# TACC/GraviT

Hardware: AMD Instinct MI355X
Metric: Mrays/s (primary+shadow) at 1080p, 10M-tri scene (higher is better)
Workload: dtype f32; 1 GPU; soup-10000000: 10000000 random triangles (Philox seed 12345, half-extent 0.005), 1920x1080, eye (.5,.5,3)->(.5,.5,.5), fov 30deg, 1 point light at the eye, depth 1 (primary + 1 shadow ray), AO off; scheduler=image, 1 domain, harness=native, settle_frames=0, normal_mode=flat

## Files before the change

### gravit_amd/capi.py

```python
import ctypes as C
import os

import numpy as np

from .layouts import HIT_DTYPE, LIGHT_DTYPE, MATERIAL_DTYPE, RAY_DTYPE

HERE = os.path.dirname(os.path.abspath(__file__))
LIB_PATH = os.environ.get("GVT_HIP_LIB") or os.path.join(HERE, "libgvt_hip.so")

ABI_VERSION = 6

SYMBOLS = [
    "gvt_hip_init", "gvt_hip_set_stream", "gvt_hip_synchronize", "gvt_hip_last_error",
    "gvt_hip_mesh_create", "gvt_hip_mesh_destroy", "gvt_hip_trace_ex", "gvt_hip_mesh_get_info", "gvt_hip_mesh_get_normals", "gvt_hip_mesh_update_vertices",
    "gvt_hip_trace", "gvt_hip_intersect", "gvt_hip_occluded",
    "gvt_hip_queue_create", "gvt_hip_queue_destroy", "gvt_hip_queue_reserve", "gvt_hip_queue_clear", "gvt_hip_queue_size",
    "gvt_hip_queue_append", "gvt_hip_queue_append_flags", "gvt_hip_abi_version", "gvt_hip_queue_export", "gvt_hip_trace_queue", "gvt_hip_trace_queue_sink",
    "gvt_hip_camera_generate",
    "gvt_hip_camera_generate_tiled",
    "gvt_hip_camera_filter",
    "gvt_hip_top_create", "gvt_hip_top_destroy", "gvt_hip_top_order", "gvt_hip_top_update", "gvt_hip_shuffle", "gvt_hip_queue_sizes",
    "gvt_hip_fb_create", "gvt_hip_fb_destroy", "gvt_hip_fb_clear", "gvt_hip_fb_download", "gvt_hip_fb_device_ptr",
    "gvt_hip_fb_write_ppm_bytes",
    "gvt_hip_profile", "gvt_hip_stats_read", "gvt_hip_stats_reset", "gvt_hip_set_option", "gvt_hip_is_experiments_build", "gvt_hip_counters_peek", "gvt_hip_visit_stats", "gvt_hip_wide_visit_stats", "gvt_hip_mesh_download_nodes", "gvt_hip_mesh_download_wide", "gvt_hip_mesh_download_clusters", "gvt_hip_mesh_upload_nodes", "gvt_hip_marked_visit_stats", "gvt_hip_image_frame",
    "gvt_hip_math_probe", "gvt_hip_ctx_create", "gvt_hip_ctx_make_current", "gvt_hip_ctx_destroy",
    "gvt_hip_comm_unique_id", "gvt_hip_comm_create", "gvt_hip_hub_create", "gvt_hip_hub_abort", "gvt_hip_hub_destroy", "gvt_hip_comm_create_local",
    "gvt_hip_comm_destroy", "gvt_hip_comm_rank", "gvt_hip_comm_world", "gvt_hip_comm_count", "gvt_hip_comm_reserved_cus", "gvt_hip_comm_set_deadline_ms", "gvt_hip_comm_selftest",
    "gvt_hip_tracer_create", "gvt_hip_tracer_destroy", "gvt_hip_tracer_set_camera", "gvt_hip_tracer_set_transforms", "gvt_hip_tracer_set_domains", "gvt_hip_tracer_frame",
    "gvt_hip_volume_create", "gvt_hip_volume_destroy", "gvt_hip_volume_get_info", "gvt_hip_volume_set_transfer", "gvt_hip_volume_trace",
    "gvt_hip_shuffle_volume", "gvt_hip_volume_frame",
    "gvt_hip_volume_set_surfaces", "gvt_hip_volume_set_lights", "gvt_hip_volume_get_crossings",
    "gvt_hip_volume_set_shading", "gvt_hip_volume_get_shading", "gvt_hip_volume_get_shaded",
    "gvt_hip_volume_update_samples",
    "gvt_hip_volume_create_typed", "gvt_hip_volume_update_samples_typed", "gvt_hip_volume_get_voxel_type",
    "gvt_hip_depth_create", "gvt_hip_depth_destroy", "gvt_hip_depth_clear", "gvt_hip_depth_upload", "gvt_hip_depth_download", "gvt_hip_depth_render",
    "gvt_hip_volume_frame_clipped", "gvt_hip_fb_composite_over",
    "gvt_hip_volume_set_subgrids", "gvt_hip_volume_get_amr_info",
    "gvt_hip_volume_march_queue", "gvt_hip_volume_camera_filter", "gvt_hip_queues_export_wire", "gvt_hip_queues_append_wire",
    "gvt_hip_volume_set_ghosts", "gvt_hip_volume_set_gradient", "gvt_hip_volume_get_gradient",
    "gvt_hip_volume_frame_fused", "gvt_hip_volume_frame_fused_shaded", "gvt_hip_volume_frame_fused_amr",
    "gvt_hip_volume_frame_shadowed",
    "gvt_hip_volume_light_grid_bake", "gvt_hip_volume_light_grid_download", "gvt_hip_volume_light_grid_info", "gvt_hip_volume_light_grid_release",
    "gvt_hip_volume_frame_fog_shadowed",
    "gvt_hip_volume_occluder_grid_bake", "gvt_hip_volume_occluder_grid_download", "gvt_hip_volume_occluder_grid_info", "gvt_hip_volume_occluder_grid_release",
    "gvt_hip_volume_frame_mesh_shadowed",
]


class GvtHipError(RuntimeError):
    pass


class MeshInfo(C.Structure):
    _fields_ = [("n_tris", C.c_uint64), ("n_verts", C.c_uint64), ("n_nodes", C.c_uint64), ("n_leaves", C.c_uint64),
                ("bbox_lo", C.c_float * 3), ("bbox_hi", C.c_float * 3), ("build_ms", C.c_float), ("max_leaf", C.c_uint32),
                ("packet", C.c_uint32), ("bytes_nodes", C.c_uint64), ("bytes_tris", C.c_uint64), ("sah_inner", C.c_float), ("pad", C.c_float)]


class CameraPod(C.Structure):
    _fields_ = [("eye", C.c_float * 3), ("focus", C.c_float * 3), ("up", C.c_float * 3), ("fov", C.c_float), ("width", C.c_int32),
                ("height", C.c_int32), ("samples", C.c_int32), ("depth", C.c_int32), ("jitter_window_size", C.c_float)]


class FrameStats(C.Structure):
    _fields_ = [("rounds", C.c_uint64), ("chains", C.c_uint64), ("host_syncs", C.c_uint64), ("rays_sent", C.c_uint64),
                ("rays_closest", C.c_uint64), ("rays_any", C.c_uint64), ("packets_bailed", C.c_uint64), ("bytes_sent", C.c_uint64),
                ("ms_chain", C.c_double), ("ms_announce", C.c_double), ("ms_payload", C.c_double), ("ms_composite", C.c_double), ("ms_host_wait", C.c_double),
                ("exchanges", C.c_uint64), ("rays_inline", C.c_uint64), ("early_deposit_launches", C.c_uint64)]

    def as_dict(self):
        return {k: getattr(self, k) for k, _ in self._fields_}


class VolumeInfo(C.Structure):
    _fields_ = [("box_lo", C.c_float * 3), ("box_hi", C.c_float * 3), ("dt", C.c_float), ("value_min", C.c_float), ("value_max", C.c_float),
                ("blocks", C.c_int32 * 3), ("pad", C.c_float), ("n_blocks", C.c_uint64), ("n_blocks_empty", C.c_uint64),
                ("samples_marched", C.c_uint64), ("samples_gathered", C.c_uint64)]

    def as_dict(self):
        return {k: (list(getattr(self, k)) if k in ("box_lo", "box_hi", "blocks") else getattr(self, k)) for k, _ in self._fields_ if k != "pad"}


class SubgridPod(C.Structure):
    _fields_ = [("parent", C.c_int32), ("ratio", C.c_int32), ("lo", C.c_int32 * 3), ("cells", C.c_int32 * 3)]


class VolumeAmrInfo(C.Structure):
    _fields_ = [("n_subgrids", C.c_int32), ("n_levels", C.c_int32), ("subgrid_bytes", C.c_uint64), ("samples_refined", C.c_uint64),
                ("amr_marches", C.c_uint64)]

    def as_dict(self):
        return {k: getattr(self, k) for k, _ in self._fields_}


class VolumeFusedStats(C.Structure):
    _fields_ = [("fused", C.c_uint32), ("pad", C.c_uint32), ("samples_marched", C.c_uint64), ("samples_gathered", C.c_uint64),
                ("brick_visits", C.c_uint64), ("rays_deposited", C.c_uint64), ("adapter_calls", C.c_uint64)]

    def as_dict(self):
        return {k: getattr(self, k) for k, _ in self._fields_ if k != "pad"}


class VolumeFusedShadedStats(C.Structure):
    _fields_ = [("fused", C.c_uint32), ("features", C.c_uint32), ("samples_marched", C.c_uint64), ("samples_gathered", C.c_uint64),
                ("brick_visits", C.c_uint64), ("rays_deposited", C.c_uint64), ("adapter_calls", C.c_uint64), ("crossings_rendered", C.c_uint64),
                ("samples_shaded", C.c_uint64)]

    def as_dict(self):
        return {k: getattr(self, k) for k, _ in self._fields_}


class VolumeFusedAmrStats(C.Structure):
    _fields_ = VolumeFusedShadedStats._fields_ + [("samples_refined", C.c_uint64), ("amr_bricks", C.c_uint32), ("pad", C.c_uint32)]

    def as_dict(self):
        return {k: getattr(self, k) for k, _ in self._fields_ if k != "pad"}


class VolumeShadowParams(C.Structure):
    _fields_ = [("flags", C.c_uint32), ("bias", C.c_int32)]


class VolumeShadowStats(C.Structure):
    _fields_ = VolumeFusedShadedStats._fields_ + [("shadowed", C.c_uint32), ("pad", C.c_uint32), ("shadow_rays", C.c_uint64), ("shadow_brick_visits", C.c_uint64),
                                                  ("shadow_crossings", C.c_uint64), ("shadow_samples_marched", C.c_uint64), ("shadow_samples_gathered", C.c_uint64)]

    def as_dict(self):
        return {k: getattr(self, k) for k, _ in self._fields_ if k != "pad"}


class VolumeLightGridParams(C.Structure):
    _fields_ = [("flags", C.c_uint32), ("bias", C.c_int32)]


class VolumeLightGridStats(C.Structure):
    _fields_ = [("rays", C.c_uint64), ("samples_marched", C.c_uint64), ("samples_gathered", C.c_uint64), ("crossings", C.c_uint64), ("bytes", C.c_uint64),
                ("ms", C.c_float), ("pad", C.c_uint32)]

    def as_dict(self):
        return {k: getattr(self, k) for k, _ in self._fields_ if k != "pad"}


class VolumeLightGridState(C.Structure):
    _fields_ = [("present", C.c_uint32), ("current", C.c_uint32), ("n_planes", C.c_int32), ("bias", C.c_int32), ("bytes", C.c_uint64)]

    def as_dict(self):
        return {k: getattr(self, k) for k, _ in self._fields_}


class VolumeFogShadowStats(C.Structure):
    _fields_ = VolumeShadowStats._fields_ + [("fog_samples_shadowed", C.c_uint64)]
# ... 203 lines not shown
```

### gravit_amd/csrc/api.hip

```cpp
#include <atomic>
#include <chrono>
#include <cmath>
#include <cstdlib>
#include <condition_variable>
#include <functional>
#include <mutex>
#include <new>
#include <thread>

#include "gvt_internal.h"

size_t trav_spill_ints_per_thread();
int trav_block_threads();
void abi_pool_destroy(void *);

static thread_local std::string g_err;
static Ctx g_default_ctx;
static thread_local Ctx *tl_ctx = nullptr;
#define g_ctx (gctx())
Ctx &gctx() { return tl_ctx ? *tl_ctx : g_default_ctx; }

void set_error(const char *fmt, ...) {
  char buf[1024];
  va_list ap;
// ... 134 lines not shown
  C.scratch_bytes[slot] = want;
  return C.scratch[slot];
}

void scratch_release(ScratchSlot slot) {
  Ctx &C = g_ctx;
  if (!C.scratch[slot]) return;
  hipStreamSynchronize(C.stream);
  hipFree(C.scratch[slot]);
  C.scratch[slot] = nullptr;
  C.scratch_bytes[slot] = 0;
}

ProfScope::ProfScope(int c) : cls(c) {
  Ctx &C = g_ctx;
  if (!C.profile || (C.profile == 2 && c != KC_CLOSEST && c != KC_ANY && c != KC_LONG) || (C.profile == 3 && c != KC_CLOSEST) || (C.profile == 4 && c != KC_ANY)) return;
  auto take = [&]() {
    hipEvent_t e;
    if (!C.event_pool.empty()) { e = C.event_pool.back(); C.event_pool.pop_back(); }
    else hipEventCreate(&e);
    return e;
  };
  a = take(); b = take();
  hipEventRecord(a, C.stream);
}
ProfScope::~ProfScope() {
  Ctx &C = g_ctx;
  if (!a) return;
  hipEventRecord(b, C.stream);
  C.pending.push_back({ a, b, cls });
}
static void drain_events() {
  Ctx &C = g_ctx;
  for (auto &p : C.pending) {
    hipEventSynchronize(p.b);
    float ms = 0.f;
    hipEventElapsedTime(&ms, p.a, p.b);
    double *slot[KC_COUNT] = { &C.stats.ms_closest, &C.stats.ms_any, &C.stats.ms_shade, &C.stats.ms_convert, &C.stats.ms_shuffle,
                               &C.stats.ms_camera, &C.stats.ms_build, &C.stats.ms_sort, &C.stats.ms_long };
    *slot[p.cls] += ms;
    C.event_pool.push_back(p.a);
    C.event_pool.push_back(p.b);
  }
  C.pending.clear();
}
extern "C" int gvt_hip_profile(int enable) {
  if (ensure_init()) return GVT_HIP_ERR_NODEVICE;
  drain_events();
  g_ctx.profile = enable < 0 ? 0 : enable;
  return 0;
}
extern "C" int gvt_hip_stats_read(gvt_hip_stats *out) {
  if (!out) { set_error("stats_read: null"); return GVT_HIP_ERR_INVALID; }
  if (ensure_init()) return GVT_HIP_ERR_NODEVICE;
  HIPCHK(hipStreamSynchronize(g_ctx.stream));
  drain_events();
  *out = g_ctx.stats;
  return 0;
}
extern "C" int gvt_hip_stats_reset(void) {
  if (ensure_init()) return GVT_HIP_ERR_NODEVICE;
  drain_events();
  g_ctx.stats = gvt_hip_stats{};
  return 0;
}

namespace {
struct KnobDef { const char *name; int Knobs::*field; int lo, hi; bool shipped; };
const KnobDef g_knobs[] = {
  { "skip_known", &Knobs::skip_known, 0, 1, true },           { "frame_timing", &Knobs::frame_timing, 0, 1, true },
  { "term_sink", &Knobs::term_sink, 0, 1, true },
  { "sort_rays", &Knobs::sort_rays, 0, 1, true },             { "leaf_max", &Knobs::leaf_max, 1, 4, true },
  { "long_steps", &Knobs::long_steps, 0, 1 << 20, true },     { "small_rays", &Knobs::small_rays, 0, 1 << 30, true },
  { "finish_rays", &Knobs::finish_rays, 0, 1 << 30, true },   { "round_room_mb", &Knobs::round_room_mb, 0, 1 << 30, true },
  { "abi_lanes", &Knobs::abi_lanes_n, 0, 8, true },           { "abi_chunk", &Knobs::abi_chunk, 16384, 1 << 30, true },
  { "inject_fail_tick", &Knobs::inject_fail_tick, -1, 1 << 30, true },
  { "long_min_rays", &Knobs::long_min_rays, 0, 1 << 30, true }, { "long_auto", &Knobs::long_auto, 0, 1, true },
  { "finish_auto", &Knobs::finish_auto, 0, 1, true },
  { "payload_overlap_kb", &Knobs::payload_overlap_kb, 0, 1 << 30, true },
  { "packet", &Knobs::packet, 0, 2, true },                   { "packet_sah_max", &Knobs::packet_sah_max, 0, 1 << 30, true },
  { "packet_min_rays", &Knobs::packet_min_rays, 0, 1 << 30, true },
  { "shadow_order", &Knobs::shadow_order, 0, 1, true },       { "shadow_order_min_rays", &Knobs::shadow_order_min_rays, 0, 1 << 30, true },
  { "xcd_stripes", &Knobs::xcd_stripes, 0, 1, true },           { "early_deposit", &Knobs::early_deposit, 0, 1, true },

  { "inline_kb", &Knobs::inline_kb, 0, 1024, true },          { "comm_cus", &Knobs::comm_cus, 0, 128, true },
  { "comm_stream", &Knobs::comm_stream, 0, 1, true },         { "spec_ticks", &Knobs::spec_ticks, 0, 1, true },
  { "finish_clusters", &Knobs::finish_clusters, 0, 1, true }, { "hop_local", &Knobs::hop_local, 0, 3, true },
  { "occluder_chunk", &Knobs::occluder_chunk, 0, 1 << 24, true },
  { "blocks_per_cu", &Knobs::blocks_per_cu, 1, 8, false },    { "blocks_per_cu_closest", &Knobs::blocks_per_cu_closest, 0, 8, false },
  { "refill_min", &Knobs::refill_min, 1, 64, false },         { "inner_min", &Knobs::inner_min, 1, 64, false },
  { "share", &Knobs::share, 0, 1, false },                    { "share_min_rays", &Knobs::share_min_rays, 0, 1 << 30, false },
  { "sort_gather", &Knobs::sort_gather, 0, 1, false },        { "sort_bits", &Knobs::sort_bits, 8, 32, false },
  { "long_steps_drain", &Knobs::long_steps_drain, 0, 1 << 20, false }, { "long_save", &Knobs::long_save, 0, 1, false },
  { "lean_frame", &Knobs::lean_frame, 0, 1, false },          { "report_poll", &Knobs::report_poll, 0, 1, false },
  { "first_round_async", &Knobs::first_round_async, 0, 1, false }, { "wave_single", &Knobs::wave_single, 0, 1, false },
  { "shadow_direct", &Knobs::shadow_direct, 0, 1, false },    { "top_ordered", &Knobs::top_ordered, 0, 1, false },
  { "top_lds", &Knobs::top_lds, 0, 1, false },                { "camera_tile", &Knobs::camera_tile, 0, 8, false },
  { "abi_pipe_min", &Knobs::abi_pipe_min, 0, 1 << 30, false },
  { "shadow_cls_lo", &Knobs::shadow_cls_lo, 0, 255, false },  { "shadow_cls_shift", &Knobs::shadow_cls_shift, 0, 6, false },
};
}

extern "C" int gvt_hip_set_option(const char *name, int value) {
  if (!name) { set_error("set_option: null name"); return GVT_HIP_ERR_INVALID; }
  if (!std::strcmp(name, "defaults")) { static_cast<Knobs &>(g_ctx) = Knobs{}; return 0; }
  for (const KnobDef &k : g_knobs) {
    if (std::strcmp(name, k.name)) continue;
    if (value < k.lo || value > k.hi) { set_error("set_option: %s must be %d..%d", name, k.lo, k.hi); return GVT_HIP_ERR_INVALID; }
    if (!std::strcmp(name, "camera_tile") && value != 0 && value != 8) { set_error("camera_tile: 0 or 8"); return GVT_HIP_ERR_INVALID; }
#ifndef GVT_EXPERIMENTS
    if (!k.shipped && value != Knobs{}.*(k.field)) {
      set_error("set_option: %s=%d needs the experiments build of the library (libgvt_hip_exp.so); the shipped library carries its measured-best value %d", name, value,
                Knobs{}.*(k.field));
      return GVT_HIP_ERR_INVALID;
    }
#endif
    static_cast<Knobs &>(g_ctx).*(k.field) = value;
    return 0;
  }
  set_error("set_option: unknown option '%s'", name);
  return GVT_HIP_ERR_INVALID;
}

static void default_material(gvt_hip_material *m) {
  std::memset(m, 0, sizeof *m);
  m->type = 0;
  m->kd[0] = m->kd[1] = m->kd[2] = .5f;
  m->ks[0] = m->ks[1] = m->ks[2] = .5f;
  m->alpha = 1.f;
  m->eta[0] = .19f; m->eta[1] = 1.45f; m->eta[2] = 1.50f;
  m->k[0] = 3.06f; m->k[1] = 2.40f; m->k[2] = 1.88f;
  m->roughness = 0.05f;
}

static void generate_normals(const float *verts, size_t nV, const int32_t *tris, size_t nT, std::vector<float> &normals) {
  normals.assign(nV * 3, 0.0f);
  for (size_t i = 0; i < nT; i++) {
    int I = tris[3 * i], J = tris[3 * i + 1], K = tris[3 * i + 2];
    V3 a = ld3(verts + 3 * I), b = ld3(verts + 3 * J), c = ld3(verts + 3 * K);
    V3 u = sub3(b, a), v = sub3(c, a), n;
    n.x = u.y * v.z - u.z * v.y;
    n.y = u.z * v.x - u.x * v.z;
    n.z = u.x * v.y - u.y * v.x;
    n = norm3(n);
    int idx[3] = { I, J, K };
    for (int k = 0; k < 3; k++) {
      float *d = &normals[3 * idx[k]];
      d[0] += n.x; d[1] += n.y; d[2] += n.z;
    }
  }
  for (size_t i = 0; i < nV; i++) {
    V3 n = norm3(ld3(&normals[3 * i]));
    normals[3 * i] = n.x; normals[3 * i + 1] = n.y; normals[3 * i + 2] = n.z;
  }
}

template <typename T> static bool upload(T **dst, const T *src, size_t n) {
  *dst = nullptr;
  if (hipMalloc((void **)dst, sizeof(T) * (n ? n : 1)) != hipSuccess) return false;
  if (n && hipMemcpy(*dst, src, sizeof(T) * n, hipMemcpyHostToDevice) != hipSuccess) return false;
  return true;
}

extern "C" gvt_hip_mesh *gvt_hip_mesh_create(const float *verts, size_t nV, const int32_t *tris, size_t nT, const float *vnormals,
                                             const float *vcolors, const gvt_hip_material *materials, size_t nMat,
                                             const int32_t *face_mat, const gvt_hip_material *mesh_mat) {
// ... 557 lines not shown
```

### gravit_amd/csrc/domain.hip

```cpp
#include <dlfcn.h>
#include <rccl/rccl.h>

#include <atomic>
#include <condition_variable>
#include <memory>
#include <mutex>

#include <chrono>
#include <thread>

#include "gvt_internal.h"

int shuffle_async(gvt_hip_top *T, gvt_hip_queue *q_in, size_t n_ub, const int *from_arr, int from, gvt_hip_queue *const *queues, const uint8_t *keep_mask,
                  gvt_hip_fb *fb, unsigned *d_overflow, const void *d_qdesc);
int shuffle_exact(gvt_hip_top *T, gvt_hip_queue *q_in, const int *from_arr, int from, gvt_hip_queue *const *queues, gvt_hip_fb *fb);
int camera_one_instance_async(gvt_hip_top *T, const gvt_hip_camera *cam, int tile, gvt_hip_queue *q, gvt_hip_fb *fb, unsigned *d_overflow, unsigned *d_moved_count, unsigned *row_rays);
int camera_filter_async(gvt_hip_top *T, const gvt_hip_camera *cam, int tile, gvt_hip_queue *const *queues, const uint8_t *keep_mask, unsigned *d_overflow,
                        size_t first, size_t count, bool rect = false, unsigned *row_rays = nullptr);
size_t camera_instance_bound(gvt_hip_top *T, const gvt_hip_camera *cam, int tile, size_t inst);

namespace {
struct Rccl {
  void *lib = nullptr;
  ncclResult_t (*GetUniqueId)(ncclUniqueId *) = nullptr;
// ... 1189 lines not shown
  R->layout_agreed = true;
  return 0;
}

extern "C" int gvt_hip_tracer_frame(gvt_hip_tracer *R, int flags, gvt_hip_frame_stats *out) {
  if (ensure_init()) return GVT_HIP_ERR_NODEVICE;
  if (!R) { set_error("tracer_frame: null"); return GVT_HIP_ERR_INVALID; }
  Ctx &C = gctx();
  hipStream_t st = C.stream;
  const size_t nI = R->n_inst, row = ANN_HEAD + nI;
  const bool bsp = (flags & GVT_HIP_FRAME_BSP) != 0;
  const bool image_split = (flags & GVT_HIP_FRAME_IMAGE) != 0 && R->world > 1;
  int rc0 = 0;
  if (image_split)
    for (size_t i = 0; i < nI; i++)
      if (!R->meshes[i]) { set_error("tracer_frame: GVT_HIP_FRAME_IMAGE needs every instance's mesh on every rank (instance %zu has none)", i); return GVT_HIP_ERR_INVALID; }
  if (R->world > 1 && R->inl_bytes != ((size_t)C.inline_kb << 10)) {
    HIPCHK(hipStreamSynchronize(st));
    if ((rc0 = tracer_alloc_tables(R))) return rc0;
  }
  if ((rc0 = tracer_handshake(R))) return rc0;
  if (R->comm) { R->comm->ms_host_wait = 0.0; R->comm->groups = 0; }
  const int world_saved = R->world;
  std::vector<uint8_t> owned_saved = R->owned;
  struct Restore {
    gvt_hip_tracer *R; int world; const std::vector<uint8_t> *owned;
    ~Restore() { R->world = world; R->owned = *owned; }
  } restore{ R, world_saved, &owned_saved };
  gvt_hip_frame_stats S{};
  int rc;
  const auto frame_t0 = std::chrono::steady_clock::now();
  if (R->frame_no == 0) {
    R->surfaces = true;
    for (size_t i = 0; i < nI; i++) if (R->meshes[i] && !R->meshes[i]->packet_ok) R->surfaces = false;
  }
  size_t n_mine = 0;
  for (size_t i = 0; i < nI && n_mine < 2; i++) n_mine += (R->world == 1 || image_split || R->owned[i]) ? 1 : 0;
  const bool hop_ok = C.hop_local > 0 && C.term_sink && !C.skip_known && n_mine > 1;
  const bool one_rank_many = R->world == 1 && nI > 1;
  unsigned allowed = 0;
  for (int v = 0; v < 6; v++) {
    const bool f = (v & 1) != 0;
    const int h = v >> 1;
    if (f ? C.finish_rays <= 0 : (C.finish_rays > 0 && !(C.finish_auto && one_rank_many))) continue;
    if (!hop_ok) { if (h) continue; }
    else if (C.hop_local == 2) { if (h != 2) continue; }
    else if (C.hop_local == 3) { if (h != 1) continue; }
    else if (!one_rank_many && h != (R->surfaces ? 2 : 0)) continue;
    allowed |= 1u << v;
  }
  int n_allowed = 0, route_list[6] = { 0, 0, 0, 0, 0, 0 };
  for (int v = 0; v < 6; v++) if ((allowed >> v) & 1u) route_list[n_allowed++] = v;
  const bool fin_auto = n_allowed > 1;
  int fin_variant = route_list[n_allowed - 1];
  {
    const int h0 = !hop_ok ? 0 : C.hop_local == 2 ? 2 : C.hop_local == 3 ? 1 : R->surfaces ? 2 : 0, f0 = C.finish_rays > 0 ? 1 : 0;
    for (int k = 0; k < n_allowed; k++) if ((route_list[k] >> 1) == h0 && (route_list[k] & 1) == f0) fin_variant = route_list[k];
  }
  if (fin_auto && R->frame_no >= 2) {
    if ((R->frame_no & 2047u) == 0 || (R->fin_choice >= 0 && !((allowed >> R->fin_choice) & 1u))) {
      R->fin_choice = -1;
      for (int v = 0; v < 6; v++) { R->fin_n[v] = 0; R->fin_best[v] = 1e30; }
    }
    if (R->fin_choice >= 0) fin_variant = R->fin_choice;
    else {
      int pick = fin_variant;
      for (int k = 0; k < n_allowed; k++) if (R->fin_n[route_list[k]] < R->fin_n[pick]) pick = route_list[k];
      fin_variant = pick;
    }
  }
  R->fin_limit = (fin_variant & 1) ? C.finish_rays : 0;
  R->hop_now = fin_variant >> 1;
  R->fin_eligible = false;
  struct LongOverride { Ctx &C; ~LongOverride() { C.long_steps_override = 0; } } long_override{ C };
  C.long_steps_override = (C.long_auto && C.long_steps > 0 && R->long_cur > C.long_steps) ? R->long_cur : 0;
  const bool one_shot = nI == 1 && R->world == 1 && C.term_sink && C.wave_single && R->meshes[0] && C.first_round_async;
  const bool lean = one_shot && C.lean_frame && R->fb->w == R->cam.width && R->fb->h == R->cam.height;
  for (size_t i = 0; i < nI; i++) R->queues[i]->size = 0;
  R->q_moved->size = 0;
  R->sizes_exact = true; R->spec_enqueued_last = false;
  R->cam_row_rays = 0u;
  bool first_on_device = false;
  R->fb_fresh = true;
  const uint64_t early0 = C.early_deposit_launches;
  if (!lean) {
    if ((rc = gvt_hip_fb_clear(R->fb))) return rc;
    k_zero_totals<<<(unsigned)std::max<size_t>(1, (nI + 255) / 256), 256, 0, st>>>(C.d_counters, R->d_overflow, R->fb->w, R->fb->h, R->d_count_ptr, (int)nI);
  }
  if (one_shot) {
    const size_t n_cam = (size_t)R->cam.width * R->cam.height * R->cam.samples * R->cam.samples;
    const int passes0 = R->cam.depth > 1 ? R->cam.depth : 1;
    if ((rc = queue_reserve(R->queues[0], n_cam * (size_t)(1 + (int)R->lights.size() * passes0)))) return rc;
    if (lean) { if ((rc = camera_one_instance_async(R->top, &R->cam, C.camera_tile, R->queues[0], R->fb, R->d_overflow, R->q_moved->d_count, &R->cam_row_rays))) return rc; }
    else if ((rc = camera_filter_async(R->top, &R->cam, C.camera_tile, R->queues.data(), nullptr, R->d_overflow, 0, 0, false, &R->cam_row_rays))) return rc;
    R->present[0] = n_cam;
    R->queues[0]->size = n_cam;
    if ((rc = local_chain(R, nullptr, &S.chains, true, true, lean, lean))) return rc;
    if ((rc = round_report(R, false, &S.host_syncs, lean))) return rc;
  } else if (image_split) {
    const size_t n_cam = (size_t)R->cam.width * R->cam.height * R->cam.samples * R->cam.samples;
    const size_t portion = n_cam / (size_t)R->world, first = (size_t)R->rank * portion;
    const size_t count = (R->rank + 1 == R->world) ? n_cam - first : portion;
    for (size_t i = 0; i < nI; i++) if ((rc = queue_reserve(R->queues[i], count))) return rc;
    if ((rc = camera_filter_async(R->top, &R->cam, C.camera_tile, R->queues.data(), nullptr, R->d_overflow, first, count))) return rc;
    std::fill(R->owned.begin(), R->owned.end(), (uint8_t)1);
    R->world = 1;
    if ((rc = round_report(R, false, &S.host_syncs))) return rc;
  } else {
    const uint8_t *keep = R->world > 1 ? R->owned.data() : nullptr;
    const size_t n_cam = (size_t)R->cam.width * R->cam.height * R->cam.samples * R->cam.samples;
    bool on_device = C.first_round_async && C.term_sink && nI <= 16;
    std::vector<size_t> room(nI, 0);
    if (on_device) {
      size_t sum = 0;
      for (size_t i = 0; i < nI; i++) {
        if (keep && !keep[i]) continue;
        if (!R->meshes[i]) { on_device = false; break; }
        room[i] = camera_instance_bound(R->top, &R->cam, C.camera_tile, i);
        sum += room[i];
      }
      if (sum > 2 * n_cam) on_device = false;
    }
    if (on_device) {
      for (size_t i = 0; i < nI; i++) if (room[i] && (rc = queue_reserve(R->queues[i], room[i]))) return rc;
      if ((rc = camera_filter_async(R->top, &R->cam, C.camera_tile, R->queues.data(), keep, R->d_overflow, 0, 0, true, &R->cam_row_rays))) return rc;
      for (size_t i = 0; i < nI; i++) { R->present[i] = room[i]; R->queues[i]->size = room[i]; }
      first_on_device = true;
    } else {
      if ((rc = gvt_hip_camera_filter(R->top, &R->cam, C.camera_tile, R->queues.data(), keep))) return rc;
      S.host_syncs++;
      for (size_t i = 0; i < nI; i++) R->present[i] = R->queues[i]->size;
    }
  }
  std::vector<size_t> incoming(nI, 0);
  bool payload_pending = false, payload_cross = false;
  std::vector<int> pending_ann;

  auto wire_flush = [&](WireBatch &B, bool unpack) -> int {
    if (!B.n_items) return 0;
    if (unpack) k_unpack_all<<<(B.total + 255) / 256, 256, 0, st>>>(B, R->d_overflow, R->d_overflow + 11);
    else k_pack_all<<<(B.total + 255) / 256, 256, 0, st>>>(B);
    HIPCHK(hipGetLastError());
    B.n_items = 0; B.total = 0;
    return 0;
  };
  auto wire_add = [&](WireBatch &B, bool unpack, gvt_hip_queue *q, void *buf, unsigned n, int qid) -> int {
    if (B.n_items == WIRE_MAX || (unsigned long long)B.total + 2ull + 20ull * n > 0xf0000000ull) { int rc_ = wire_flush(B, unpack); if (rc_) return rc_; }
    WireItem &I = B.it[B.n_items];
    I.planes = q->d_planes; I.cap = q->cap; I.count = q->d_count; I.buf = (unsigned *)buf; I.n = n; I.qid = qid; I.dword0 = B.total; I.prior = 0u;
    if (unpack) for (int k = 0; k < B.n_items; k++) if (B.it[k].qid == qid) I.prior += B.it[k].n;
    B.n_items++; B.total += 2u + 20u * n;
    return 0;
  };
  auto unpack_pending = [&]() -> int {
    if (!payload_pending) return 0;
    if (payload_cross) HIPCHK(hipStreamWaitEvent(st, R->ev_recv, 0));
    WireBatch B;
    B.n_items = 0; B.total = 0;
    int rc_;
    for (int p = 0; p < R->world; p++) {
      if (p == R->rank) continue;
      const int *a = pending_ann.data() + (size_t)p * row;
      if (a[10]) continue;
      char *src = (char *)R->recv_buf[p];
      size_t off = 0;
      for (size_t i = 0; i < nI; i++) {
        const unsigned n = (unsigned)a[ANN_HEAD + i];
// ... 162 lines not shown
      if ((rc = comm_reduce_sum(K, R->fb->d_rgba, (size_t)R->fb->w * R->fb->h * 4, 0))) return rc;
    } else if (R->rank != 0) {
      const int *bb = (const int *)(R->h_report + nI + 6);
      const int w = bb[2] - bb[0], h = bb[3] - bb[1];
      if (w > 0 && h > 0) {
        const size_t bytes = (size_t)w * h * 16;
        if ((rc = grow(&R->send_buf[0], &R->send_cap[0], bytes))) return rc;
        k_rect<false><<<(unsigned)(((size_t)w * h + 255) / 256), 256, 0, st>>>((float4 *)R->fb->d_rgba, W, bb[0], bb[1], w, h, (float4 *)R->send_buf[0]);
        HIPCHK(hipGetLastError());
        if (K->stream != st) { HIPCHK(hipEventRecord(R->ev_compute, st)); HIPCHK(hipStreamWaitEvent(K->stream, R->ev_compute, 0)); }
        comm_group_begin(K);
        comm_send(K, R->send_buf[0], bytes, 0);
        if ((rc = comm_group_end(K))) return rc;
      }
    } else {
      if (K->stream != st) { HIPCHK(hipEventRecord(R->ev_compute, st)); HIPCHK(hipStreamWaitEvent(K->stream, R->ev_compute, 0)); }
      comm_group_begin(K);
      for (int p = 1; p < R->world; p++) {
        const int *bb = R->h_ann_in + (size_t)p * row + 4;
        const int w = bb[2] - bb[0], h = bb[3] - bb[1];
        if (w <= 0 || h <= 0) continue;
        const size_t bytes = (size_t)w * h * 16;
        if ((rc = grow(&R->recv_buf[p], &R->recv_cap[p], bytes))) return rc;
        comm_recv(K, R->recv_buf[p], bytes, p);
      }
      if ((rc = comm_group_end(K))) return rc;
      for (int p = 1; p < R->world; p++) {
        const int *bb = R->h_ann_in + (size_t)p * row + 4;
        const int w = bb[2] - bb[0], h = bb[3] - bb[1];
        if (w <= 0 || h <= 0) continue;
        k_rect<true><<<(unsigned)(((size_t)w * h + 255) / 256), 256, 0, K->stream>>>((float4 *)R->fb->d_rgba, W, bb[0], bb[1], w, h, (float4 *)R->recv_buf[p]);
      }
      HIPCHK(hipGetLastError());
    }
    HIPCHK(hipEventRecord(R->ev_comm, K->stream));
    if (K->stream != st) HIPCHK(hipStreamWaitEvent(st, R->ev_comm, 0));
    if ((rc = bounded_event_wait(K, R->ev_comm, "the framebuffer composite"))) return rc;
    S.host_syncs++;
    if (C.frame_timing) { float ms = 0.f; if (hipEventElapsedTime(&ms, R->ev_comp0, R->ev_comm) == hipSuccess) S.ms_composite += ms; }
  }
  if (R->comm) { S.ms_host_wait = R->comm->ms_host_wait; S.exchanges = R->comm->groups; }
  if (spec_trace && multi) R->comp_us += std::chrono::duration<double, std::micro>(std::chrono::steady_clock::now() - t_mark).count();
  const unsigned *tail = R->h_report + nI;
  S.rays_closest = (uint64_t)tail[0] | ((uint64_t)tail[1] << 32);
  S.rays_any = (uint64_t)tail[2] | ((uint64_t)tail[3] << 32);
  S.packets_bailed = tail[10];
  if (C.long_auto && C.long_steps > 0 && S.rays_closest >= 65536) {
    const double frac = (double)tail[11] / (double)S.rays_closest;
    int cur = std::max(R->long_cur, C.long_steps);
    if (frac > 0.01) cur = std::min(1024, cur + cur / 2);
    else if (frac > 0.003) cur = std::min(1024, cur + cur / 4);
    else if (frac < 0.0005) cur = std::max(C.long_steps, cur - cur / 5);
    R->long_cur = cur;
  }
  C.stats.rays_closest += S.rays_closest;
  C.stats.rays_any += S.rays_any;
  if (fin_auto && R->frame_no >= 2 && R->fin_choice < 0) {
    const double ms = std::chrono::duration<double, std::milli>(std::chrono::steady_clock::now() - frame_t0).count();
    R->fin_best[fin_variant] = std::min(R->fin_best[fin_variant], ms);
    R->fin_n[fin_variant]++;
    R->fin_probe++;
    bool once = true;
    double lead = 1e30;
    for (int k = 0; k < n_allowed; k++) { once = once && R->fin_n[route_list[k]] >= 1; lead = std::min(lead, R->fin_best[route_list[k]]); }
    if (once) for (int k = 0; k < n_allowed; k++) if (R->fin_best[route_list[k]] > 1.3 * lead) R->fin_n[route_list[k]] = std::max(R->fin_n[route_list[k]], 3);
    bool all = true;
    int best = route_list[0];
    for (int k = 0; k < n_allowed; k++) {
      all = all && R->fin_n[route_list[k]] >= 3;
      if (R->fin_best[route_list[k]] < R->fin_best[best] || (R->fin_best[route_list[k]] == R->fin_best[best] && route_list[k] > best)) best = route_list[k];
    }
    if (all) {
      R->fin_choice = best;
      if (getenv("GVT_HIP_ROUTE_TRACE")) {
        fprintf(stderr, "[tracer] frame %llu: route settled -- k_finish %d, hops %s; fastest frame per route timed, ms:", (unsigned long long)R->frame_no, best & 1,
                (best >> 1) == 0 ? "never" : (best >> 1) == 1 ? "early" : "always");
        for (int k = 0; k < n_allowed; k++) fprintf(stderr, " [k_finish %d hops %d] %.3f", route_list[k] & 1, route_list[k] >> 1, R->fin_best[route_list[k]]);
        fprintf(stderr, "\n");
      }
    }
  }
  R->frame_no++;
  S.early_deposit_launches = C.early_deposit_launches - early0;
  if (out) *out = S;
  return 0;
}
```

### gravit_amd/csrc/gvt_device.h

```cpp
#pragma once
#include <hip/hip_runtime.h>
#include <stdint.h>

#include "../../include/gvt_hip.h"
#define GVT_MATH_FN __host__ __device__ static inline
#include "../../include/gvt_math.h"
#include "xcd_stripes.h"

#define GVT_RAY_EPSILON 1.e-6f
#define GVT_FLT_MAX 3.402823466e+38f
#define GVT_FLT_EPSILON 1.192092896e-07f

enum CounterWord {
  CW_WORK = 0,
  CW_SHADOW = 1,
  CW_BOUNCE_A = 2,
  CW_BOUNCE_B = 5,
  CW_LONG = 3,
  CW_LONG_WORK = 4,
  CW_PKT_RETRY = 6,
  CW_TRAV_OVF = 8,
  CW_PACKETS = 9,
  CW_TOT_CLOSEST = 16,
  CW_TOT_ANY = 18,
  CW_LONG_FRAME = 20,
  CW_MERGED_N = 22,
  CW_SHADOW_CLS = 24,
  CW_PEEK = 32,
  CW_WORK_XCD = 64,
  CW_LINE = 32,
  CW_COUNT = CW_WORK_XCD + 7 * CW_LINE
};
__host__ __device__ constexpr unsigned cw_work_stripe(unsigned x) { return x ? (unsigned)CW_WORK_XCD - CW_WORK + (x - 1u) * CW_LINE : 0u; }
__device__ inline void cw_zero_work(unsigned *c) {
#pragma unroll
  for (unsigned x = 0; x < 8u; x++) c[CW_WORK + cw_work_stripe(x)] = 0u;
}
enum { TOT_CLOSEST = 0, TOT_ANY = 1 };
__host__ __device__ inline unsigned long long *cw_totals(unsigned *c) { return (unsigned long long *)(c + CW_TOT_CLOSEST); }
__host__ __device__ inline int cw_bounce(int pass) { return (pass & 1) ? CW_BOUNCE_B : CW_BOUNCE_A; }
static_assert(CW_TOT_ANY == CW_TOT_CLOSEST + 2 && CW_LONG_FRAME == CW_TOT_ANY + 2, "k_cam1_count clears the totals and the parked total as one run of five words");
static_assert(CW_LINE * sizeof(unsigned) == 128 && CW_WORK_XCD % CW_LINE == 0 && CW_WORK + cw_work_stripe(7) < CW_COUNT, "every stripe's work counter has a 128-byte line of its own inside the allocation");
static_assert(CW_SHADOW_CLS + 8 <= CW_WORK_XCD && CW_PEEK <= CW_WORK_XCD, "no named counter word shares a line with the counters of stripes 1..7 (stripe 0 keeps CW_WORK's)");
static_assert(CW_LONG_WORK == 4 && CW_BOUNCE_A < 5 && CW_LONG < 5, "k_trace_begin / launch_closest zero words 0..4 as one run");

struct V3 {
  float x, y, z;
};
__host__ __device__ inline V3 mk3(float x, float y, float z) { V3 r; r.x = x; r.y = y; r.z = z; return r; }
__host__ __device__ inline V3 ld3(const float *p) { return mk3(p[0], p[1], p[2]); }
__host__ __device__ inline V3 add3(V3 a, V3 b) { return mk3(a.x + b.x, a.y + b.y, a.z + b.z); }
__host__ __device__ inline V3 sub3(V3 a, V3 b) { return mk3(a.x - b.x, a.y - b.y, a.z - b.z); }
__host__ __device__ inline V3 mul3(V3 a, V3 b) { return mk3(a.x * b.x, a.y * b.y, a.z * b.z); }
__host__ __device__ inline V3 scl3(V3 a, float s) { return mk3(a.x * s, a.y * s, a.z * s); }
__host__ __device__ inline V3 neg3(V3 a) { return mk3(-a.x, -a.y, -a.z); }
__host__ __device__ inline float dot3(V3 a, V3 b) { V3 t = mul3(a, b); return t.x + t.y + t.z; }
__host__ __device__ inline V3 cross3(V3 x, V3 y) {
  return mk3(x.y * y.z - y.y * x.z, x.z * y.x - y.z * x.x, x.x * y.y - y.x * x.y);
}
__host__ __device__ inline float len3(V3 a) { return sqrtf(dot3(a, a)); }
__host__ __device__ inline V3 norm3(V3 a) { return scl3(a, 1.0f / sqrtf(dot3(a, a))); }

struct Mat4 {
  float m[16];
};
struct Mat3 {
  float n[9];
};
__host__ __device__ inline V3 xfm_point(const Mat4 &M, V3 p) {
  const float *m = M.m;
  return mk3((m[0] * p.x + m[4] * p.y) + (m[8] * p.z + m[12] * 1.0f), (m[1] * p.x + m[5] * p.y) + (m[9] * p.z + m[13] * 1.0f),
             (m[2] * p.x + m[6] * p.y) + (m[10] * p.z + m[14] * 1.0f));
}
__host__ __device__ inline V3 xfm_vector(const Mat4 &M, V3 d) {
  const float *m = M.m;
  return mk3((m[0] * d.x + m[4] * d.y) + (m[8] * d.z + m[12] * 0.0f), (m[1] * d.x + m[5] * d.y) + (m[9] * d.z + m[13] * 0.0f),
             (m[2] * d.x + m[6] * d.y) + (m[10] * d.z + m[14] * 0.0f));
}
__host__ __device__ inline V3 mat3_mul(const Mat3 &N, V3 v) {
  const float *n = N.n;
  return mk3(n[0] * v.x + n[3] * v.y + n[6] * v.z, n[1] * v.x + n[4] * v.y + n[7] * v.z, n[2] * v.x + n[5] * v.y + n[8] * v.z);
}

struct RayPlanes {
  float4 *p0, *p1, *p2, *p3;
  uint32_t *p4;
  uint32_t *p5;
};
#define GVT_QUEUE_BYTES_PER_RAY (4 * sizeof(float4) + 4 * sizeof(uint32_t))
__host__ __device__ inline RayPlanes make_planes(float4 *base, size_t cap) {
  RayPlanes r;
  r.p0 = base; r.p1 = base + cap; r.p2 = base + 2 * cap; r.p3 = base + 3 * cap; r.p4 = (uint32_t *)(base + 4 * cap); r.p5 = r.p4 + cap;
  return r;
}

struct RayRec {
  V3 o; float t_min;
  V3 d; float t_max;
  V3 c; float t;
  int id, depth; float w; int type;
  uint32_t rng;
  uint32_t km[3];
};
__device__ inline RayRec load_ray(const RayPlanes &q, size_t i) {
  float4 a = q.p0[i], b = q.p1[i], c = q.p2[i], d = q.p3[i];
  RayRec r;
  r.o = mk3(a.x, a.y, a.z); r.t_min = a.w;
  r.d = mk3(b.x, b.y, b.z); r.t_max = b.w;
  r.c = mk3(c.x, c.y, c.z); r.t = c.w;
  r.id = __float_as_int(d.x); r.depth = __float_as_int(d.y); r.w = d.z; r.type = __float_as_int(d.w);
  r.rng = q.p4 ? q.p4[i] : 0u;
  if (q.p5) { r.km[0] = q.p5[3 * i]; r.km[1] = q.p5[3 * i + 1]; r.km[2] = q.p5[3 * i + 2]; }
  else { r.km[0] = 0u; r.km[1] = 0u; r.km[2] = 0u; }
  return r;
}
__device__ inline void store_ray(const RayPlanes &q, size_t i, const RayRec &r) {
  q.p0[i] = make_float4(r.o.x, r.o.y, r.o.z, r.t_min);
  q.p1[i] = make_float4(r.d.x, r.d.y, r.d.z, r.t_max);
  q.p2[i] = make_float4(r.c.x, r.c.y, r.c.z, r.t);
  q.p3[i] = make_float4(__int_as_float(r.id), __int_as_float(r.depth), r.w, __int_as_float(r.type));
  if (q.p4) q.p4[i] = r.rng;
  if (q.p5) { q.p5[3 * i] = r.km[0]; q.p5[3 * i + 1] = r.km[1]; q.p5[3 * i + 2] = r.km[2]; }
}
__device__ inline void store_no_known(const RayPlanes &q, size_t i) { if (q.p5) { q.p5[3 * i] = 0u; q.p5[3 * i + 1] = 0u; q.p5[3 * i + 2] = 0u; } }

struct BvhNode {
  float4 n0, n1, n2, n3;
};
#ifndef GVT_LEAF_MAX
#define GVT_LEAF_MAX 2
#endif
#define GVT_NODE4_F4 4
#define GVT_EMPTY_REF (-1)
__host__ __device__ inline int leaf_ref(uint32_t first, uint32_t count) { return ~(int)((first << 3) | count); }

__device__ inline bool tri_test(V3 O, V3 D, V3 v0, V3 e1, V3 e2, float tnear, float &t, float &u, float &v) {
  V3 Ng = cross3(e1, e2);
  V3 C = sub3(v0, O);
  V3 R = cross3(D, C);
  float den = dot3(Ng, D);
  float absDen = fabsf(den);
  float sgn = (den < 0.f) ? -1.f : 1.f;
  float U = dot3(R, e2) * sgn;
  float V = dot3(R, e1) * sgn;
// ... 213 lines not shown
```

### gravit_amd/csrc/gvt_internal.h

```cpp
#pragma once
#include <hip/hip_runtime.h>

#include <cstdarg>
#include <cstdio>
#include <cstring>
#include <string>
#include <vector>

#include "gvt_device.h"

enum KernelClass { KC_CLOSEST = 0, KC_ANY, KC_SHADE, KC_CONVERT, KC_SHUFFLE, KC_CAMERA, KC_BUILD, KC_SORT, KC_LONG, KC_COUNT };

struct PendingEvent {
  hipEvent_t a, b;
  int cls;
};

#define SHADOW_CLASSES 8
static_assert(CW_SHADOW_CLS + SHADOW_CLASSES <= CW_PEEK, "the class counts are read through gvt_hip_counters_peek");
static_assert(CW_SHADOW_CLS + SHADOW_CLASSES <= CW_COUNT && CW_PEEK <= CW_COUNT, "every named counter word lies inside the allocation");

enum ScratchSlot {
  SCR_GENERAL,
  SCR_SHADOW,
  SCR_IDX_A,
  SCR_IDX_B,
  SCR_LIGHTS,
  SCR_NEXT_INST,
  SCR_NEXT_T,
  SCR_SORT_KEYS_IN, SCR_SORT_KEYS_OUT, SCR_SORT_VALS_IN, SCR_SORT_VALS_OUT,
  SCR_SORT_TEMP, SCR_SORT_GATHER,
  SCR_BLOCK_COUNTS,
  SCR_LONG,
  SCR_SHADOW_INST, SCR_OUT_FROM,
  SCR_PKT_RETRY,
  SCR_STEPS,
  SCR_VOL_WORK, SCR_VOL_OVF,
  SCR_VOL_RANGES,
  SCR_BUILD,
  SCR_HOP,
  SCR_WIRE_TABLE,
  SCR_VOL_KEEP,
  SCR_VOL_BRICKS, SCR_VOL_FUSED,
  SCR_VOL_GRIDS,
  SCR_VOL_OCC_RAYS, SCR_VOL_OCC,
  SCR_VOL_GHOSTS,
  SCR_VOL_AMR,
  SCRATCH_COUNT
};
struct Knobs {
  int blocks_per_cu = 4;
  int blocks_per_cu_closest = 5;
  int refill_min = 16;
  int inner_min = 32;
  int share = 1;
  int share_min_rays = 131072;
  int sort_rays = 0;
  int sort_gather = 0;
  int sort_bits = 20;
  int long_steps = 96;
  int long_steps_drain = 0;
  int long_save = 1;
  int long_min_rays = 65536;
  int packet = 1;
  int shadow_order = 1;
  int shadow_cls_lo = 24, shadow_cls_shift = 3;
  int xcd_stripes = 1;
  int early_deposit = 1;
  int shadow_order_min_rays = 262144;
  int packet_min_rays = 524288;
  int packet_sah_max = 128;
  int round_room_mb = 16384;
  int finish_rays = 32768;
  int finish_auto = 1;
  int small_rays = 4096;
  int abi_lanes_n = 4;
  int abi_chunk = 262144;
  int abi_pipe_min = 131072;
  int lean_frame = 1;
  int skip_known = 0;
  int long_auto = 1;
  int payload_overlap_kb = 1024;
  int inline_kb = 16;
  int comm_cus = 0;
  int hop_local = 1;
  int finish_clusters = 1;
  int spec_ticks = 1;
  int comm_stream = 0;
  int frame_timing = 0;
  int inject_fail_tick = -1;
  int report_poll = 1;
  int first_round_async = 1;
  int wave_single = 1;
  int shadow_direct = 1;
  int term_sink = 1;
  int camera_tile = 8;
  int top_ordered = 1;
  int top_lds = 1;
  int leaf_max = 2;
  int occluder_chunk = 0;
};

struct Ctx : Knobs {
  bool ready = false;
  int device = -1;
  hipStream_t own_stream = nullptr;
  hipStream_t stream = nullptr;
  int profile = 0;
  int long_steps_override = 0;
  std::vector<PendingEvent> pending;
  std::vector<hipEvent_t> event_pool;
  gvt_hip_stats stats{};
  int n_cu = 256;
  uint64_t early_deposit_launches = 0;
  bool shadow_order_denied = false;
  int cu_reserved = 0;
  int trav_blocks = 0;
  int *d_spill = nullptr;
  unsigned *d_counters = nullptr;
  unsigned *h_pinned = nullptr;
  void *h_wire = nullptr;
  hipEvent_t wire_ev = nullptr;
  bool wire_busy = false;
  void *scratch[SCRATCH_COUNT] = { nullptr };
  size_t scratch_bytes[SCRATCH_COUNT] = { 0 };
  std::vector<unsigned char> lights_cached;
  const void *lights_cached_dst = nullptr;
  gvt_hip_queue *abi_qin = nullptr, *abi_qout = nullptr;
  std::vector<Ctx *> abi_lanes;
  void *abi_pool = nullptr;
};
Ctx &gctx();
void set_error(const char *fmt, ...);
int ensure_init();
inline bool staging_queues(Ctx &C) {
  if (!C.abi_qin) { C.abi_qin = gvt_hip_queue_create(0); C.abi_qout = gvt_hip_queue_create(0); }
  return C.abi_qin && C.abi_qout;
}
void *scratch_get(ScratchSlot slot, size_t bytes);
void scratch_release(ScratchSlot slot);

#define HIPCHK(expr)                                                                              \
  do {                                                                                            \
    hipError_t _e = (expr);                                                                       \
    if (_e != hipSuccess) {                                                                       \
      set_error("%s failed: %s (%s:%d)", #expr, hipGetErrorString(_e), __FILE__, __LINE__);       \
      return GVT_HIP_ERR_DEVICE;                                                                  \
    }                                                                                             \
  } while (0)

struct ProfScope {
  int cls;
  hipEvent_t a = nullptr, b = nullptr;
  explicit ProfScope(int cls);
  ~ProfScope();
};

struct gvt_hip_mesh {
  size_t nV = 0, nT = 0;
  float *d_verts = nullptr;
  int *d_tris = nullptr;
  float *d_normals = nullptr;
  float *d_vcolors = nullptr;
  gvt_hip_material *d_materials = nullptr;
  size_t nMat = 0;
  int *d_face_mat = nullptr;
  gvt_hip_material mesh_mat;
  BvhNode *d_nodes = nullptr;
  size_t nNodes = 0;
  float4 *d_tri = nullptr;
  unsigned *d_slot_of = nullptr;
  uint4 *d_nodes4 = nullptr;
  size_t nNodes4 = 0;
  std::vector<unsigned> levels4;
  uint4 *d_nodes4c = nullptr;
  int root_entry4c = 0;
  int leaf_max = 2;
  size_t nLeaves = 0;
  float lo[3] = { 0, 0, 0 }, hi[3] = { 0, 0, 0 };
  float build_ms = 0.f;
  float sah_inner = 0.f;
  bool packet_ok = false;
  uint2 *d_range2 = nullptr;
  uint2 *d_range4 = nullptr;
  unsigned *d_vlist = nullptr;
  unsigned *d_vstart = nullptr;
};

struct gvt_hip_queue {
  float4 *d_planes = nullptr;
  size_t cap = 0;
  size_t size = 0;
  unsigned *d_count = nullptr;
};

struct gvt_hip_top {
  size_t n = 0;
// ... 143 lines not shown
```

### gravit_amd/csrc/shade.inc

```
__device__ inline V3 light_contribution(const gvt_hip_light &L, V3 hit, V3 samplePos) {
  V3 c = ld3(L.color);
  if (L.type == GVT_HIP_LIGHT_AMBIENT) return c;
  V3 p = (L.type == GVT_HIP_LIGHT_AREA) ? samplePos : ld3(L.position);
  float distance = 1.f / len3(sub3(p, hit));
  distance = (distance > 1.f) ? 1.f : distance;
  return scl3(c, distance);
}

__device__ inline V3 area_light_position(const gvt_hip_light &L, uint32_t &seed) {
  V3 v = ld3(L.normal), u, w;
  if (v.x == 0.f && v.y == 1.f && v.z == 0.f) {
    u = mk3(1, 0, 0); w = mk3(0, 0, 1);
  } else {
    const V3 up = mk3(0, 1, 0);
    u.x = up.y * v.z - v.y * up.z; u.y = up.z * v.x - v.z * up.x; u.z = up.x * v.y - v.x * up.y;
    w.x = v.y * u.z - u.y * v.z; w.y = v.z * u.x - u.z * v.x; w.z = v.x * u.y - u.x * v.y;
  }
  float xLocation = (float)(((double)gvt_fastrand_lcg(seed, 0, 1) - 0.5) * (double)L.width);
  float zLocation = (float)(((double)gvt_fastrand_lcg(seed, 0, 1) - 0.5) * (double)L.height);
  float xCoord = xLocation * u.x + zLocation * w.x;
  float yCoord = xLocation * u.y + zLocation * w.y;
  float zCoord = xLocation * u.z + zLocation * w.z;
  return mk3(L.position[0] + xCoord, L.position[1] + yCoord, L.position[2] + zCoord);
}
// ... 64 lines not shown
      const float cosThetaO = dot3(wo, N), cosThetaI = dot3(wi, N);
      if (!(cosThetaI <= 0.0f || cosThetaO <= 0.0f)) {
        const V3 s_ = add3(wi, wo);
        const V3 wh = scl3(s_, 1.0f / sqrtf(dot3(s_, s_)));
        const float cosThetaH = dot3(wh, N);
        const float cosTheta = dot3(wi, wh);
        const float cosi = cosTheta, c2 = cosi * cosi;
        const V3 tmp = add3(mul3(m.eta, m.eta), mul3(m.k, m.k));
        const V3 two_eta_c = scl3(scl3(m.eta, 2.0f), cosi);
        const V3 one = mk3(1.0f, 1.0f, 1.0f), vc2 = mk3(c2, c2, c2);
        const V3 num1 = add3(sub3(scl3(tmp, c2), two_eta_c), one), den1 = add3(add3(scl3(tmp, c2), two_eta_c), one);
        const V3 num2 = add3(sub3(tmp, two_eta_c), vc2), den2 = add3(add3(tmp, two_eta_c), vc2);
        const V3 Rpar = mk3(num1.x / den1.x, num1.y / den1.y, num1.z / den1.z);
        const V3 Rper = mk3(num2.x / den2.x, num2.y / den2.y, num2.z / den2.z);
        const V3 F = scl3(add3(Rpar, Rper), 0.5f);
        const float D = (expo + 2) * (1.0f / (2.0f * 3.14159265358979323846f)) * powf(fabsf(cosThetaH), expo);
        const float g1 = 2.0f * cosThetaH * cosThetaO / cosTheta, g2 = 2.0f * cosThetaH * cosThetaI / cosTheta;
        const float gm = (g1 < g2) ? g1 : g2;
        const float G = (1.0f < gm) ? 1.0f : gm;
        r = scl3(scl3(scl3(mul3(ks, F), D), G), 1.0f / (4.0f * cosThetaO));
      }
    }
    color = scl3(scl3(r, 2.f), ray.w);
  } else {
    color = mk3(0, 0, 0);
  }
  color = mul3(color, Li);
  float c[3] = { color.x, color.y, color.z };
  for (int i = 0; i < 3; i++) {
    float a = (c[i] < 0.f) ? 0.f : c[i];
    c[i] = (1.f < a) ? 1.f : a;
  }
  out = mk3(c[0], c[1], c[2]);
  return true;
}

__device__ inline V3 cos_weighted_dir(V3 n, uint32_t &seed) {
  float Xi1 = gvt_fastrand01(seed);
  float Xi2 = gvt_fastrand01(seed);
  float theta = (float)gvt_acos(__builtin_sqrt(1.0 - (double)Xi1));
  float phi = (float)(2.0 * 3.1415926535897932384626433832795 * (double)Xi2);
  float xs = gvt_sinf(theta) * gvt_cosf(phi);
  float ys = gvt_cosf(theta);
  float zs = gvt_sinf(theta) * gvt_sinf(phi);
  V3 y = n, h = y;
  if (fabsf(h.x) <= fabsf(h.y) && fabsf(h.x) <= fabsf(h.z)) h.x = 1.0f;
  else if (fabsf(h.y) <= fabsf(h.x) && fabsf(h.y) <= fabsf(h.z)) h.y = 1.0f;
  else h.z = 1.0f;
  V3 x = cross3(h, y);
  V3 z = cross3(x, y);
  V3 d = add3(add3(scl3(x, xs), scl3(y, ys)), scl3(z, zs));
  return norm3(d);
}

struct ShadeArgs {
  RayPlanes in;
  const unsigned *idx;
  unsigned n;
  unsigned long long index_base;
  const gvt_hip_hit *hits;
  int first_pass;
  int carried_rng;
  RayPlanes out; unsigned *out_count;
  RayPlanes shadow; unsigned *shadow_count;
  unsigned *next_idx; unsigned *next_count;
  const gvt_hip_light *lights;
  Mat3 normi;
  int normal_mode, n_lights;
  uint32_t seed;
  unsigned *zero_word;
  TermSink sink;
  int update_in_place;
  const unsigned *n_dev;
  WaveSet W;
  const int *hop_inst;
  int *out_from;
  int *shadow_inst;
  unsigned shadow_stride;
  const unsigned char *steps;
  unsigned *cls_cnt;
  unsigned cls_stride;
  int cls_lo, cls_shift;
  int early_deposit;
};

__device__ __forceinline__ void store_shadow_early(const ShadeArgs &A, unsigned slot, const RayRec &s) {
  A.shadow.p0[slot] = make_float4(s.o.x, s.o.y, s.o.z, s.t_min);
  A.shadow.p1[slot] = make_float4(s.d.x, s.d.y, s.d.z, s.t_max);
  const bool dep = len3(s.c) > 0.f && (unsigned)s.id < A.sink.n_pix;
  if (dep) {
    const V3 cw = scl3(s.c, s.w);
    ((float4 *)A.sink.fb)[(unsigned)s.id] = make_float4(0.0f + cw.x, 0.0f + cw.y, 0.0f + cw.z, 1.0f);
  }
  ((uint32_t *)A.shadow.p2)[slot] = dep ? (uint32_t)s.id : 0xffffffffu;
}

__device__ __forceinline__ unsigned shadow_class(int steps, int lo, int shift) {
  const int c = (steps - lo) >> shift;
  return (unsigned)(c < 0 ? 0 : (c > SHADOW_CLASSES - 1 ? SHADOW_CLASSES - 1 : c));
}

#define SHADE_BLOCK 512
template <bool MULTI, bool LEAN = false>
__global__ __launch_bounds__(SHADE_BLOCK, 4) void k_shade(ShadeArgs A, MeshView M1) {
  __shared__ unsigned sh_alloc[2 * (2 + 64)];
  __shared__ unsigned sh_cls[2 * SHADOW_CLASSES];
  for (int k = threadIdx.x; k < 2 * (2 + 64); k += SHADE_BLOCK) sh_alloc[k] = 0u;
  if (threadIdx.x < 2 * SHADOW_CLASSES) sh_cls[threadIdx.x] = 0u;
  __syncthreads();
  const unsigned j = blockIdx.x * blockDim.x + threadIdx.x;
  if (j == 0 && A.zero_word) *A.zero_word = 0u;
  const unsigned n = A.n_dev ? *A.n_dev : A.n;
  const bool in_range = j < n;
  __shared__ unsigned sh_wcls[SHADE_BLOCK / 64];
  if (!MULTI && A.cls_cnt) {
    int st = in_range ? (int)A.steps[j] : 0;
    for (int o = 32; o >= 1; o >>= 1) st = max(st, __shfl_xor(st, o));
    if (lane_id() == 0) sh_wcls[threadIdx.x >> 6] = shadow_class(st, A.cls_lo, A.cls_shift);
  }
  unsigned i = in_range ? (A.idx ? A.idx[j] : j) : 0u;
  const unsigned gi = i;
  RayPlanes in = A.in;
  const MeshView *M = &M1;
  Mat3 normi = A.normi;
  int inst = A.sink.from;
  if (MULTI && in_range) {
    const WaveSeg sg = A.W.segs[wave_find_seg(A.W, i)];
    in = make_planes(sg.planes, sg.cap);
    i -= sg.begin;
    inst = sg.inst;
    if (A.hop_inst) { const int h_ = A.hop_inst[gi]; if (h_ >= 0) inst = h_; }
    M = &A.W.insts[inst].mv;
    normi = A.W.insts[inst].normi;
  }
  RayRec r;
  gvt_hip_hit h;
  h.prim = -1; h.t = 0.f; h.u = 0.f; h.v = 0.f;
  bool miss = false, shaded = false, bounce = false;
  uint32_t g_seed = 0;
  V3 N = mk3(0, 0, 0);
  MatEval me = mat_eval(M->mat);
  if (in_range) {
    r = load_ray(in, i);
    h = A.hits[j];
    if (!LEAN) g_seed = (A.first_pass && (!A.carried_rng || r.rng == 0u)) ? ray_stream_seed(A.seed, A.index_base + gi) : r.rng;
    if (h.prim < 0) {
      miss = true;
    } else if (r.type != 1) {
      shaded = true;
      float t = h.t;
      r.t = t;
      const float4 *sl = M->slots + 4 * (size_t)M->slot_of[h.prim];
      const float4 s0 = sl[0], s1 = sl[1], s2 = sl[2], s3 = sl[3];
      const V3 v0 = mk3(s0.x, s0.y, s0.z), v1 = mk3(s1.w, s2.w, s3.x), v2 = mk3(s3.y, s3.z, s3.w);
      int ia = 0, ib = 0, ic = 0;
      if (A.normal_mode == GVT_HIP_NORMALS_SMOOTH || (!LEAN && M->vcolors)) { ia = M->tris[3 * h.prim]; ib = M->tris[3 * h.prim + 1]; ic = M->tris[3 * h.prim + 2]; }
      const V3 negNg = cross3(sub3(v1, v0), sub3(v2, v0));
      const V3 normalflat = norm3(mat3_mul(normi, negNg));
      if (A.normal_mode == GVT_HIP_NORMALS_SMOOTH) {
        const V3 a = ld3(M->normals + 3 * ib), b = ld3(M->normals + 3 * ic), c = ld3(M->normals + 3 * ia);
        const V3 mn = add3(add3(scl3(a, h.u), scl3(b, h.v)), scl3(c, 1.0f - h.u - h.v));
        N = norm3(mat3_mul(normi, mn));
      } else {
        N = normalflat;
      }
      if (dot3(neg3(r.d), normalflat) <= 0.f) N = neg3(N);
      if (LEAN) {
      } else if (M->vcolors) {
        const V3 c0 = ld3(M->vcolors + 3 * ia), c1 = ld3(M->vcolors + 3 * ib), c2 = ld3(M->vcolors + 3 * ic);
        me.kd = add3(add3(scl3(c0, 1.f - h.u - h.v), scl3(c1, h.u)), scl3(c2, h.v));
        me.type = 0; me.ks = mk3(.5f, .5f, .5f); me.alpha = 1.f;
      } else if (M->face_mat && M->face_mat[h.prim] >= 0 && (unsigned)M->face_mat[h.prim] < M->n_mat) {
        me = mat_eval(M->materials[M->face_mat[h.prim]]);
      }
      if (r.type == 2) {
        t = (t > 1) ? 1.f / t : t;
        r.w = r.w * t;
      }
    }
  }
  if (!(LEAN && !MULTI)) {
    bool forward = miss;
    if (miss && A.sink.fb) {
      float ret_t;
      const float4 a = make_float4(r.o.x, r.o.y, r.o.z, r.t_min), b = make_float4(r.d.x, r.d.y, r.d.z, r.t_max);
      if (top_nearest(a, b, A.sink.top, inst, ret_t) < 0) {
        forward = false;
        deposit_shadow(A.sink.fb, A.sink.n_pix, r.type, r.c, r.w, (unsigned)r.id);
      }
    }
    const unsigned slot = block_alloc(A.out_count, forward, &sh_alloc[0]);
    if (forward) { store_ray(A.out, slot, r); if (MULTI) A.out_from[slot] = inst; }
  }
  for (int li = 0; li < A.n_lights; li++) {
    bool emit = false;
    RayRec s;
    if (shaded) {
      const gvt_hip_light L = A.lights[li];
      const V3 lightPos = (!LEAN && L.type == GVT_HIP_LIGHT_AREA) ? area_light_position(L, g_seed) : ld3(L.position);
      V3 c;
      if (shade<LEAN>(me, r, N, L, lightPos, c)) {
        emit = true;
        const float multiplier = 1.0f - GVT_RAY_EPSILON * 16;
        const float t_shadow = multiplier * r.t;
        const V3 origin = add3(r.o, scl3(r.d, t_shadow));
        const V3 dir = sub3(lightPos, origin);
        s.o = origin; s.t_min = GVT_RAY_EPSILON;
        s.d = norm3(dir);
        s.t_max = 3.0f;
        s.c = c; s.t = r.t;
        s.id = r.id; s.depth = r.depth; s.w = r.w; s.type = 1;
        s.rng = 0u;
        s.km[0] = 0u; s.km[1] = 0u; s.km[2] = 0u;
      }
    }
    if (A.shadow_stride) {
      if (j < A.shadow_stride) {
        const unsigned slot = (unsigned)li * A.shadow_stride + j;
        A.shadow_inst[slot] = emit ? (MULTI ? inst : 0) : -1;
        if (emit) store_ray(A.shadow, slot, s);
      }
    } else if (!MULTI && A.cls_cnt) {
      const unsigned cls = (unsigned)__builtin_amdgcn_readfirstlane((int)sh_wcls[threadIdx.x >> 6]);
      const unsigned long long mask = ballot64(emit);
      unsigned woff = 0;
      if (mask) {
        if ((int)lane_id() == __ffsll((long long)mask) - 1) woff = atomicAdd(&sh_cls[cls], (unsigned)__popcll(mask));
        woff = (unsigned)__builtin_amdgcn_readlane((int)woff, __ffsll((long long)mask) - 1);
      }
      __syncthreads();
      if (threadIdx.x < SHADOW_CLASSES && sh_cls[threadIdx.x]) sh_cls[SHADOW_CLASSES + threadIdx.x] = atomicAdd(&A.cls_cnt[threadIdx.x], sh_cls[threadIdx.x]);
      __syncthreads();
      if (emit) {
        const unsigned slot = cls * A.cls_stride + sh_cls[SHADOW_CLASSES + cls] + woff + lanes_below(mask);
        if (LEAN && A.early_deposit) store_shadow_early(A, slot, s);
        else store_ray(A.shadow, slot, s);
      }
    } else {
      const unsigned slot = block_alloc(A.shadow_count, emit, &sh_alloc[2 * (2 + li)]);
      if (emit) {
// ... 32 lines not shown
```

### gravit_amd/csrc/trace.hip

```cpp
#include "gvt_internal.h"

#ifndef TRAV_BLOCK
#define TRAV_BLOCK 256
#endif
#define TRAV_WAVES_PER_BLOCK (TRAV_BLOCK / 64)
#ifndef TRAV_STACK
#define TRAV_STACK 24
#endif
#ifndef KT_BLOCKS_CLOSEST
#define KT_BLOCKS_CLOSEST 5
#endif
#ifndef RETIRE_BATCH
#define RETIRE_BATCH 1
#endif
#ifndef KT_BLOCKS_ANY
#define KT_BLOCKS_ANY 4
#endif
#define TRAV_SPILL 128

namespace {

struct Trav {
  const BvhNode *__restrict__ nodes;
  const float4 *__restrict__ tris;
// ... 103 lines not shown
  MeshView mv;
  mv.slots = M->d_tri; mv.slot_of = M->d_slot_of; mv.verts = M->d_verts; mv.tris = M->d_tris; mv.normals = M->d_normals; mv.vcolors = M->d_vcolors;
  mv.materials = M->d_materials; mv.n_mat = (unsigned)M->nMat; mv.face_mat = M->d_face_mat; mv.mat = M->mesh_mat;
  return mv;
}
bool walks_packets(const Ctx &C, const gvt_hip_mesh *M, size_t n) { return C.packet == 2 || (C.packet == 1 && M->packet_ok && n >= (size_t)C.packet_min_rays); }
bool plain_lambert(const gvt_hip_mesh *M) { return !M->d_vcolors && !M->d_face_mat && M->mesh_mat.type == 0; }
bool no_area_light(const gvt_hip_light *lights, int nL) { return std::all_of(lights, lights + nL, [](const gvt_hip_light &l) { return l.type != GVT_HIP_LIGHT_AREA; }); }

static bool lights_cached_at(const Ctx &C, const void *dst, const gvt_hip_light *lights_host, int nL) {
  const size_t bytes = sizeof(gvt_hip_light) * (size_t)nL;
  return C.lights_cached_dst == dst && C.lights_cached.size() == bytes && std::memcmp(C.lights_cached.data(), lights_host, bytes) == 0;
}
bool finish_lights_resident(const gvt_hip_light *lights_host, int nL) {
  Ctx &C = gctx();
  return !nL || (C.scratch[SCR_LIGHTS] && lights_cached_at(C, C.scratch[SCR_LIGHTS], lights_host, nL));
}
static int lights_on_device(const gvt_hip_light *lights_host, int nL, gvt_hip_light **d_lights, bool may_upload = true) {
  Ctx &C = gctx();
  *d_lights = (gvt_hip_light *)scratch_get(SCR_LIGHTS, sizeof(gvt_hip_light) * (nL > 0 ? nL : 1));
  if (!*d_lights) return GVT_HIP_ERR_DEVICE;
  if (!nL || lights_cached_at(C, *d_lights, lights_host, nL)) return 0;
  if (!may_upload) { set_error("finish_round: a speculative launch needs the light list resident"); return GVT_HIP_ERR_INVALID; }
  const size_t bytes = sizeof(gvt_hip_light) * (size_t)nL;
  C.lights_cached.assign((const unsigned char *)lights_host, (const unsigned char *)lights_host + bytes);
  C.lights_cached_dst = *d_lights;
  HIPCHK(hipMemcpyAsync(*d_lights, C.lights_cached.data(), bytes, hipMemcpyHostToDevice, C.stream));
  HIPCHK(hipStreamSynchronize(C.stream));
  return 0;
}

struct ChainBufs {
  gvt_hip_hit *hits; unsigned *idx_a, *idx_b; gvt_hip_light *lights;
  size_t shadow_cap; RayPlanes shadow;
  unsigned char *steps;
};
static int chain_bufs(ChainBufs &B, size_t n, int nL, const gvt_hip_light *lights_host, size_t ordered_slots = 0) {
  Ctx &C = gctx();
  B.hits = (gvt_hip_hit *)scratch_get(SCR_GENERAL, sizeof(gvt_hip_hit) * n);
  B.shadow_cap = n * (size_t)(nL > 0 ? nL : 1);
  size_t slots = ordered_slots ? ordered_slots : B.shadow_cap;
  float4 *d_shadow = (float4 *)scratch_get(SCR_SHADOW, sizeof(float4) * 4 * slots);
  B.steps = (ordered_slots && d_shadow) ? (unsigned char *)scratch_get(SCR_STEPS, n) : nullptr;
  if (ordered_slots && (!d_shadow || !B.steps)) {
    (void)hipGetLastError();
    C.shadow_order_denied = true;
    B.steps = nullptr;
    slots = B.shadow_cap;
    d_shadow = (float4 *)scratch_get(SCR_SHADOW, sizeof(float4) * 4 * slots);
  }
  B.idx_a = (unsigned *)scratch_get(SCR_IDX_A, sizeof(unsigned) * n);
  B.idx_b = (unsigned *)scratch_get(SCR_IDX_B, sizeof(unsigned) * n);
  if (!B.hits || !d_shadow || !B.idx_a || !B.idx_b) return GVT_HIP_ERR_DEVICE;
  B.shadow = make_planes(d_shadow, slots);
  B.shadow.p4 = nullptr; B.shadow.p5 = nullptr;
  return lights_on_device(lights_host, nL, &B.lights);
}

static int sort_ray_list(const gvt_hip_mesh *M, RayPlanes q, const unsigned **idx, size_t n, size_t n_cap, const Mat4 &minv, const unsigned *n_dev = nullptr) {
  Ctx &C = gctx();
  unsigned *k_in = (unsigned *)scratch_get(SCR_SORT_KEYS_IN, sizeof(unsigned) * n_cap), *k_out = (unsigned *)scratch_get(SCR_SORT_KEYS_OUT, sizeof(unsigned) * n_cap);
  unsigned *v_in = (unsigned *)scratch_get(SCR_SORT_VALS_IN, sizeof(unsigned) * n_cap), *v_out = (unsigned *)scratch_get(SCR_SORT_VALS_OUT, sizeof(unsigned) * n_cap);
  if (!k_in || !k_out || !v_in || !v_out) return GVT_HIP_ERR_DEVICE;
  const float ex = M->hi[0] - M->lo[0], ey = M->hi[1] - M->lo[1], ez = M->hi[2] - M->lo[2];
  const float3 blo = make_float3(M->lo[0], M->lo[1], M->lo[2]);
  const float3 inv = make_float3(ex > 0 ? 1.f / ex : 0.f, ey > 0 ? 1.f / ey : 0.f, ez > 0 ? 1.f / ez : 0.f);
  {
    ProfScope ps(KC_SORT);
    k_ray_keys<<<blocks_for(n), 256, 0, C.stream>>>(q, *idx, (unsigned)n, minv, blo, inv, k_in, v_in, C.sort_bits, n_dev);
    if (int rc = sort_pairs_u32(k_in, k_out, v_in, v_out, n, C.sort_bits)) return rc;
  }
  HIPCHK(hipGetLastError());
  *idx = v_out;
  return 0;
}

struct TraceSrc { RayPlanes q; Mat4 minv; Trav T; WaveSet W; TermSink sink; MultiSrc MS; const int *hop; unsigned row; };
static unsigned stripe_arg(unsigned row) { return (gctx().xcd_stripes && row) ? row : XCD_STRIPES_OFF; }
enum StepMode { BY_LANES, BY_PACKETS, BY_WAVES };
static int wave_grid(size_t n) { return (int)std::min<size_t>((n + 3) / 4, (size_t)gctx().n_cu * 3); }

template <bool XFORM, bool MULTI>
static void closest_step(StepMode mode, const TraceSrc &S, const unsigned *idx, size_t n, const unsigned *n_dev, float tnear, gvt_hip_hit *d_hits, const LongQ &LQ,
                         LongRec *d_long, bool later_pass = false) {
  Ctx &C = gctx();
  hipStream_t st = C.stream;
  unsigned *c = C.d_counters;
  const int tail_grid = C.n_cu * 3;
  RayPlanes none{};
  if (mode == BY_PACKETS) {
    ProfScope ps(KC_CLOSEST);
    LongQ LP{ d_long, c + CW_LONG, nullptr, 0u, 0, 0 };
    if constexpr (MULTI) k_packet_multi<<<blocks_for(n), 256, 0, st>>>(S.W, (unsigned)n, n_dev, tnear, d_hits, LP, c + CW_PACKETS);
    else k_packet<false><<<blocks_for(n), 256, 0, st>>>(S.q, (unsigned)n, n_dev, S.minv, S.T, tnear, d_hits, nullptr, none, nullptr, TermSink{}, LP, nullptr, nullptr, nullptr, c + CW_PACKETS);
    k_long_closest<XFORM, MULTI><<<tail_grid, 256, 0, st>>>(S.q, d_long, c + CW_LONG, S.minv, S.T, tnear, d_hits, c + CW_LONG_WORK, S.W);
  } else if (mode == BY_WAVES) {
    ProfScope ps(KC_CLOSEST);
    k_long_seed<<<blocks_for(n), 256, 0, st>>>(d_long, c + CW_LONG, idx, (unsigned)n, n_dev);
    k_long_closest<XFORM, MULTI><<<wave_grid(n), 256, 0, st>>>(S.q, d_long, c + CW_LONG, S.minv, S.T, tnear, d_hits, c + CW_LONG_WORK, S.W, nullptr, later_pass ? S.hop : nullptr);
  } else {
    {
      ProfScope ps(KC_CLOSEST);
      launch_trace<false, XFORM, 0, MULTI>(trav_grid2(n, true), st, S.q, idx, (unsigned)n, S.minv, S.T, tnear, d_hits, nullptr, none, nullptr, c + CW_WORK, C.d_spill,
                                           C.refill_min, C.inner_min, n_dev, C.share, (unsigned)C.share_min_rays, S.sink, LQ, S.MS, MULTI ? XCD_STRIPES_OFF : stripe_arg(S.row));
    }
    if (LQ.steps) {
      ProfScope ps(KC_LONG);
      k_long_closest<XFORM, MULTI><<<tail_grid, 256, 0, st>>>(S.q, LQ.recs, LQ.count, S.minv, S.T, tnear, d_hits, c + CW_LONG_WORK, S.W, LQ.stk, S.hop);
    }
  }
}

template <bool MULTI>
static void any_step(StepMode mode, const TraceSrc &S, const unsigned *idx, size_t grid_rays, unsigned n, const unsigned *n_dev, RayPlanes out, unsigned *out_count, bool early = false) {
  Ctx &C = gctx();
  unsigned *c = C.d_counters;
  ProfScope ps(KC_ANY);
  if constexpr (!MULTI) {
    if (early && mode == BY_LANES) {
      launch_trace<true, true, 2, false>(trav_grid2(grid_rays), C.stream, S.q, idx, n, S.minv, S.T, GVT_RAY_EPSILON, nullptr, nullptr, out, out_count, c + CW_WORK, C.d_spill,
                                         C.refill_min, C.inner_min, n_dev, C.share, (unsigned)C.share_min_rays, S.sink, LongQ{}, S.MS, stripe_arg(S.row));
      C.early_deposit_launches++;
      return;
    }
  }
  if (mode == BY_WAVES) k_wave_any<MULTI><<<wave_grid(grid_rays), 256, 0, C.stream>>>(S.q, c + CW_SHADOW, S.minv, S.T, GVT_RAY_EPSILON, out, out_count, c + CW_WORK, S.sink, S.MS);
  else launch_trace<true, true, 1, MULTI>(trav_grid2(grid_rays), C.stream, S.q, idx, n, S.minv, S.T, GVT_RAY_EPSILON, nullptr, nullptr, out, out_count, c + CW_WORK, C.d_spill,
                                          C.refill_min, C.inner_min, n_dev, C.share, (unsigned)C.share_min_rays, S.sink, LongQ{}, S.MS, MULTI ? XCD_STRIPES_OFF : stripe_arg(S.row));
}

static ShadeArgs shade_args(const ChainBufs &B, const unsigned *idx, size_t n, int pass, const unsigned *n_dev, unsigned *next, unsigned *c_next, RayPlanes outp,
                            unsigned *out_count, const TraceParams &P) {
  unsigned *c = gctx().d_counters;
  ShadeArgs A{};
  A.idx = idx; A.n = (unsigned)n; A.hits = B.hits; A.first_pass = (pass == 0); A.carried_rng = 1; A.out = outp; A.out_count = out_count;
  A.shadow = B.shadow; A.shadow_count = c + CW_SHADOW; A.next_idx = next; A.next_count = c_next; A.lights = B.lights; A.normi = P.normi; A.normal_mode = P.normal_mode;
  A.n_lights = P.n_lights; A.seed = P.seed; A.zero_word = c + CW_WORK; A.sink = P.sink; A.n_dev = n_dev;
  return A;
}

template <bool MULTI>
static void shade_step(const ShadeArgs &A, const MeshView &mv, bool lean = false) {
  ProfScope ps(KC_SHADE);
  if (lean) k_shade<MULTI, true><<<blocks_for(A.n, SHADE_BLOCK), SHADE_BLOCK, 0, gctx().stream>>>(A, mv);
  else k_shade<MULTI><<<blocks_for(A.n, SHADE_BLOCK), SHADE_BLOCK, 0, gctx().stream>>>(A, mv);
}

int launch_closest(gvt_hip_mesh *M, RayPlanes q, const unsigned *idx, size_t n, bool xform, const Mat4 &minv, float tnear,
                   gvt_hip_hit *d_hits, bool counter_is_zero) {
  if (!n) return 0;
  Ctx &C = gctx();
  if (!M->d_nodes4) { int rc4 = build_nodes4(M); if (rc4) return rc4; }
  if (!counter_is_zero) HIPCHK(hipMemsetAsync(C.d_counters, 0, (CW_LONG_WORK + 1) * sizeof(unsigned), C.stream));
  LongQ LQ{};
  if (M->d_nodes4 && C.long_steps > 0 && n >= (size_t)C.long_min_rays) {
    LongRec *recs = (LongRec *)scratch_get(SCR_LONG, long_scratch_bytes(n));
    if (!recs) return GVT_HIP_ERR_DEVICE;
    LQ = long_queue(recs, n);
  }
  TraceSrc S{};
  S.q = q; S.minv = minv; S.T = Trav{ M->d_nodes, M->d_tri, M->d_nodes4 };
  if (xform) closest_step<true, false>(BY_LANES, S, idx, n, nullptr, tnear, d_hits, LQ, LQ.recs);
  else closest_step<false, false>(BY_LANES, S, idx, n, nullptr, tnear, d_hits, LQ, LQ.recs);
  HIPCHK(hipGetLastError());
  C.stats.rays_closest += n;
  C.stats.launches_closest++;
  return 0;
}

int launch_visit_stats(gvt_hip_mesh *M, RayPlanes q, size_t n, float tnear, unsigned *d_out) {
  if (!n) return 0;
  Ctx &C = gctx();
// ... 109 lines not shown
}

extern "C" int gvt_hip_math_probe(int kind, const float *in, size_t n, float *out) {
  if (ensure_init()) return GVT_HIP_ERR_NODEVICE;
  if (kind < 0 || kind > 2 || (n && (!in || !out)) || n > 0xffffffffull) { set_error("math_probe: bad argument"); return GVT_HIP_ERR_INVALID; }
  if (!n) return 0;
  Ctx &C = gctx();
  float *d = (float *)scratch_get(SCR_GENERAL, sizeof(float) * 2 * n);
  if (!d) return GVT_HIP_ERR_DEVICE;
  HIPCHK(hipMemcpyAsync(d, in, sizeof(float) * n, hipMemcpyHostToDevice, C.stream));
  k_math_probe<<<blocks_for(n), 256, 0, C.stream>>>(kind, d, (unsigned)n, d + n);
  HIPCHK(hipGetLastError());
  HIPCHK(hipMemcpyAsync(out, d + n, sizeof(float) * n, hipMemcpyDeviceToHost, C.stream));
  HIPCHK(hipStreamSynchronize(C.stream));
  return 0;
}

namespace {
__global__ void k_wave_pass_begin(unsigned *c, int pass, unsigned n_host, unsigned *out_count, const unsigned *n_dev0 = nullptr, WaveSeg *segs = nullptr, int n_seg = 0,
                                  unsigned *const *__restrict__ count_ptr = nullptr) {
  if (blockIdx.x || threadIdx.x) return;
  if (segs) {
    unsigned run = 0;
    for (int k = 0; k < n_seg; k++) { const unsigned n = *count_ptr[segs[k].inst]; segs[k].begin = run; segs[k].n = n; run += n; }
    *const_cast<unsigned *>(n_dev0) = run;
  }
  unsigned long long *tot = cw_totals(c);
  const int cur = cw_bounce(pass), prev = cw_bounce(pass + 1);
  if (pass == 0) { *out_count = 0u; c[CW_BOUNCE_A] = 0u; c[CW_BOUNCE_B] = 0u; tot[TOT_CLOSEST] += n_dev0 ? *n_dev0 : n_host; }
  else { tot[TOT_ANY] += c[CW_SHADOW]; tot[TOT_CLOSEST] += c[prev]; c[cur] = 0u; }
  c[CW_LONG_FRAME] += c[CW_LONG];
  cw_zero_work(c); c[CW_SHADOW] = 0u; c[CW_LONG] = 0u; c[CW_LONG_WORK] = 0u; c[CW_PKT_RETRY] = 0u;
  for (int k = 0; k < SHADOW_CLASSES; k++) c[CW_SHADOW_CLS + k] = 0u;
}
__global__ void k_wave_end(unsigned *c, unsigned *const *__restrict__ count_ptr, const unsigned char *__restrict__ mask, int n_inst) {
  const int i = blockIdx.x * blockDim.x + threadIdx.x;
  if (i == 0) cw_totals(c)[TOT_ANY] += c[CW_SHADOW];
  if (count_ptr && i < n_inst && mask[i]) *count_ptr[i] = 0u;
}
}

struct Chain {
  size_t n; int passes;
  const TraceParams &P; const gvt_hip_light *lights_host; gvt_hip_queue *out; RayPlanes outp;
  ChainBufs B;
  int *d_shadow_inst;
  LongRec *d_long;
  bool use_long, small;
  const unsigned *nd0;
};
struct Pass { int pass; const unsigned *n_dev, *idx; unsigned *next, *c_next; };

static int any_packets(const Chain &K, const TraceSrc &S) {
  Ctx &C = gctx();
  unsigned *c = C.d_counters;
  unsigned *d_retry = (unsigned *)scratch_get(SCR_PKT_RETRY, sizeof(unsigned) * K.B.shadow_cap);
  if (!d_retry) return GVT_HIP_ERR_DEVICE;
  ProfScope ps(KC_ANY);
  k_packet<true><<<blocks_for(K.B.shadow_cap), 256, 0, C.stream>>>(S.q, (unsigned)K.B.shadow_cap, nullptr, S.minv, S.T, GVT_RAY_EPSILON, nullptr, K.d_shadow_inst, K.outp, K.out->d_count,
                                                                 S.sink, LongQ{}, d_retry, c + CW_PKT_RETRY, cw_totals(c) + TOT_ANY, c + CW_PACKETS);
  launch_trace<true, true, 1>(trav_grid2(4096), C.stream, S.q, d_retry, 0u, S.minv, S.T, GVT_RAY_EPSILON, nullptr, nullptr, K.outp, K.out->d_count, c + CW_WORK, C.d_spill,
                              C.refill_min, C.inner_min, c + CW_PKT_RETRY, C.share, (unsigned)C.share_min_rays, S.sink, LongQ{}, MultiSrc{}, stripe_arg(0u));
  return 0;
}

static int single_pass(const Chain &K, Pass p, const WaveSingle &W1, size_t cls_stride) {
  Ctx &C = gctx();
  unsigned *c = C.d_counters;
  gvt_hip_mesh *M = W1.mesh;
  const size_t n = K.n;
  const int nL = K.P.n_lights;
  const bool have4 = M->d_nodes4 != nullptr, by_class = K.B.steps != nullptr;
  if (C.sort_rays && p.pass > 0 && n >= 8192 && have4)
    if (int rc = sort_ray_list(M, W1.planes, &p.idx, n, n, W1.minv, p.n_dev)) return rc;
  TraceSrc S{};
  S.q = W1.planes; S.minv = W1.minv; S.T = Trav{ M->d_nodes, M->d_tri, M->d_nodes4 };
  S.row = (W1.coherent && p.pass == 0 && !p.idx) ? W1.row_rays : 0u;
  LongQ LQ{};
  if (K.use_long && have4) LQ = long_queue(K.d_long, n);
  LQ.steps_out = K.B.steps;
  const bool small1 = K.small && have4;
  const bool pkt = walks_packets(C, M, n) && W1.coherent && p.pass == 0 && have4 && !small1;
  const bool pkt_any = pkt && C.packet == 2;
  closest_step<true, false>(pkt ? BY_PACKETS : small1 ? BY_WAVES : BY_LANES, S, p.idx, n, p.n_dev, GVT_RAY_EPSILON, K.B.hits, LQ, K.d_long);
  ShadeArgs A = shade_args(K.B, p.idx, n, p.pass, p.n_dev, p.next, p.c_next, K.outp, K.out->d_count, K.P);
  A.in = W1.planes; A.normi = W1.normi; A.sink.from = W1.inst;
  if (pkt_any) { A.shadow_inst = K.d_shadow_inst; A.shadow_stride = (unsigned)n; }
  A.steps = K.B.steps; A.cls_cnt = by_class ? c + CW_SHADOW_CLS : nullptr; A.cls_stride = (unsigned)cls_stride; A.cls_lo = C.shadow_cls_lo; A.cls_shift = C.shadow_cls_shift;
  const bool lean_shade = W1.coherent && p.pass == 0 && K.passes == 1 && K.P.sink.fb && K.P.sink.top.n_inst == 1 && nL >= 1 && plain_lambert(M) && no_area_light(K.lights_host, nL);
  const bool early_deposit = lean_shade && nL == 1 && K.P.one_writer && !small1 && !pkt_any && C.early_deposit;
  A.early_deposit = early_deposit ? 1 : 0;
  shade_step<false>(A, mesh_view(M), lean_shade);
  if (!nL) return 0;
  TraceSrc SA = S;
  SA.q = K.B.shadow; SA.sink = A.sink; SA.row = 0u;
  if (pkt_any) return any_packets(K, SA);
  if (by_class) { SA.MS.cls_cnt = c + CW_SHADOW_CLS; SA.MS.cls_stride = (unsigned)cls_stride; SA.MS.cls_total = c + CW_SHADOW; }
  any_step<false>(small1 ? BY_WAVES : BY_LANES, SA, nullptr, K.B.shadow_cap, 0u, by_class ? nullptr : c + CW_SHADOW, K.outp, K.out->d_count, early_deposit);
  return 0;
}

static void merged_pass(const Chain &K, const Pass &p, const WaveSet &W, const ChainOpts &O, int *d_hop, int *d_out_from) {
  Ctx &C = gctx();
  unsigned *c = C.d_counters;
  const TraceParams &P = K.P;
  const size_t n = K.n;
  const int nL = P.n_lights;
  TraceSrc S{};
  S.W = W; S.MS.W = W; S.hop = d_hop;
  if (d_hop) {
    S.sink = P.sink;
    S.MS.hop_inst = d_hop; S.MS.hop_read = p.pass > 0; S.MS.hop_owner = P.hop_owner; S.MS.hop_rank = P.hop_rank; S.MS.hop_tot = cw_totals(c) + TOT_CLOSEST; S.MS.hop_early = P.hop == 1 ? 1 : 0;
  }
  LongQ LQ{};
  if (K.use_long) LQ = long_queue(K.d_long, n);
  const bool pktm = O.multi_packets && p.pass == 0 && !K.small && p.idx == nullptr;
  closest_step<true, true>(pktm ? BY_PACKETS : K.small ? BY_WAVES : BY_LANES, S, p.idx, n, p.n_dev, GVT_RAY_EPSILON, K.B.hits, LQ, K.d_long, p.pass > 0);
  ShadeArgs A = shade_args(K.B, p.idx, n, p.pass, p.n_dev, p.next, p.c_next, K.outp, K.out->d_count, P);
  A.W = W; A.out_from = d_out_from; A.shadow_inst = K.d_shadow_inst; A.hop_inst = d_hop;
  const bool direct = C.shadow_direct && p.pass == 0 && !K.small;
  const bool direct_dev = direct && K.nd0 != nullptr && nL == 1;
  A.shadow_stride = direct ? (unsigned)n : 0u;
  const bool lean_multi = O.simple_meshes && p.pass == 0 && K.passes == 1 && nL >= 1 && no_area_light(K.lights_host, nL);
  shade_step<true>(A, MeshView{}, lean_multi);
  if (!nL) return;
  TraceSrc SA{};
  SA.q = K.B.shadow; SA.sink = P.sink;
  SA.MS = MultiSrc{ W, K.d_shadow_inst, d_out_from, direct ? cw_totals(c) + TOT_ANY : nullptr };
  if (d_hop && P.sink.fb && P.hop == 2) { SA.MS.hop_owner = P.hop_owner; SA.MS.hop_rank = P.hop_rank; SA.MS.hop_tot = cw_totals(c) + TOT_CLOSEST; }
  if (K.small) any_step<true>(BY_WAVES, SA, nullptr, K.B.shadow_cap, 0u, nullptr, K.outp, K.out->d_count);
  else any_step<true>(BY_LANES, SA, nullptr, K.B.shadow_cap, direct ? (unsigned)K.B.shadow_cap : 0u, direct ? (direct_dev ? K.nd0 : nullptr) : c + CW_SHADOW, K.outp, K.out->d_count);
}

int wave_trace_chain(const WaveSet &W, size_t n_total, int passes, gvt_hip_queue *out, int *d_out_from, const TraceParams &P,
                     const gvt_hip_light *lights_host, const WaveSingle *single, const ChainOpts &O) {
  Ctx &C = gctx();
  if (!n_total) return 0;
  hipStream_t st = C.stream;
  const int nL = P.n_lights;
  const size_t n = n_total;
  const bool by_class_wanted = single && single->mesh->d_nodes4 && C.shadow_order && nL == 1 && n >= (size_t)C.shadow_order_min_rays && n > (size_t)C.small_rays &&
                               C.long_steps > 0 && n >= (size_t)C.long_min_rays && !(walks_packets(C, single->mesh, n) && single->coherent);
  const size_t cls_stride = (n + 63) & ~(size_t)63;
  const size_t ordered_slots = (by_class_wanted && !C.shadow_order_denied && cls_stride * SHADOW_CLASSES * 64 <= ((size_t)8 << 30)) ? cls_stride * SHADOW_CLASSES : 0;
  const size_t shadow_slots = ordered_slots ? ordered_slots : n * (size_t)(nL > 0 ? nL : 1);
  if (shadow_slots >= 0xffffffffull) { set_error("round: %zu shadow slots exceed the 32-bit slot counters", shadow_slots); return GVT_HIP_ERR_INVALID; }
  Chain K{ n, passes, P, lights_host, out, make_planes(out->d_planes, out->cap) };
  int rc = chain_bufs(K.B, n, nL, lights_host, ordered_slots);
  if (rc) return rc;
  K.d_shadow_inst = (int *)scratch_get(SCR_SHADOW_INST, sizeof(int) * K.B.shadow_cap);
  K.d_long = (LongRec *)scratch_get(SCR_LONG, long_scratch_bytes(n));
  if (!K.d_shadow_inst || !K.d_long) return GVT_HIP_ERR_DEVICE;
  int *d_hop = nullptr;
  if (!single && P.hop && P.sink.fb) {
    d_hop = (int *)scratch_get(SCR_HOP, sizeof(int) * n);
    if (!d_hop) return GVT_HIP_ERR_DEVICE;
    HIPCHK(hipMemsetAsync(d_hop, 0xff, sizeof(int) * n, st));
  }
  unsigned *c = C.d_counters;
  K.use_long = C.long_steps > 0 && n >= (size_t)C.long_min_rays;
  K.small = n <= (size_t)C.small_rays;
  K.nd0 = single ? single->n_dev : O.n_dev0_multi;
  for (int pass = 0; pass < passes; pass++) {
    unsigned *const lists[2] = { K.B.idx_a, K.B.idx_b };
    const Pass p{ pass, pass ? c + cw_bounce(pass - 1) : K.nd0, pass ? lists[(pass - 1) & 1] : nullptr, lists[pass & 1], c + cw_bounce(pass) };
    if (!(pass == 0 && single && single->pass0_begun))
      k_wave_pass_begin<<<1, 64, 0, st>>>(c, pass, (unsigned)n, out->d_count, K.nd0, (pass == 0 && O.n_dev0_multi && !single) ? const_cast<WaveSeg *>(W.segs) : nullptr, W.n_seg, O.d_count_ptr);
    if (!single) merged_pass(K, p, W, O, d_hop, d_out_from);
    else if ((rc = single_pass(K, p, *single, cls_stride))) return rc;
    HIPCHK(hipGetLastError());
    C.stats.launches_closest++;
    C.stats.launches_any++;
  }
  if (!O.defer_end) k_wave_end<<<(unsigned)((std::max(O.n_inst, 1) + 255) / 256), 256, 0, st>>>(c, O.d_count_ptr, O.d_mask, O.n_inst);
// ... 148 lines not shown
```

### gravit_amd/csrc/trace_lane.inc

```
#ifndef GVT_TRI_NG_FROM_SLOT
#define GVT_TRI_NG_FROM_SLOT 1
#endif
#ifndef GVT_STAMP
#define GVT_STAMP 0
#endif
#if GVT_STAMP
__device__ unsigned long long g_stamp[24];
#endif
#ifndef TRAV_CHUNK
#define TRAV_CHUNK 256
#endif
#ifndef KT_SHARE_DELAY
#define KT_SHARE_DELAY 24
#endif
#define TRAV_DONE ((int)0x80000000)

#define LONG_SAVE 48
#define LONG_STK_CAP 65536u
struct LongRec { unsigned j, i; float bt; int bp; float bu, bv, bden; unsigned ns; };
struct LongQ {
  LongRec *recs;
  unsigned *count;
  int *stk;
  unsigned stk_cap;
  int steps;
  int steps_drain;
  unsigned char *steps_out;
};

typedef float f2 __attribute__((ext_vector_type(2)));
struct RaySlab {
  float ix, iy, iz;
  f2 ox, oy, oz;
};
__device__ __forceinline__ RaySlab make_slab(float ix, float iy, float iz, float ox, float oy, float oz) {
  RaySlab S;
  S.ix = ix; S.iy = iy; S.iz = iz;
  const float ex = fabsf(ox) * 4.76837158e-7f, ey = fabsf(oy) * 4.76837158e-7f, ez = fabsf(oz) * 4.76837158e-7f;
  S.ox = (f2){ ox + ex, ox - ex }; S.oy = (f2){ oy + ey, oy - ey }; S.oz = (f2){ oz + ez, oz - ez };
  return S;
}
__device__ __forceinline__ f2 splat2(float v) { return (f2){ v, v }; }
template <bool LIM = true>
__device__ __forceinline__ void node4_test(const uint4 *__restrict__ nd, const RaySlab &S, float lim, float tn[4], int rr[4], bool *hit = nullptr) {
  if (LIM) lim = cull_bound(lim);
  const uint4 w0 = nd[0], w1 = nd[1], w2 = nd[2], w3 = nd[3];
  const float sx = __uint_as_float(w0.w) * S.ix, sy = __uint_as_float(w3.z) * S.iy, sz = __uint_as_float(w3.w) * S.iz;
  const f2 bx = __builtin_elementwise_fma(splat2(__uint_as_float(w0.x)), splat2(S.ix), -S.ox);
  const f2 by = __builtin_elementwise_fma(splat2(__uint_as_float(w0.y)), splat2(S.iy), -S.oy);
  const f2 bz = __builtin_elementwise_fma(splat2(__uint_as_float(w0.z)), splat2(S.iz), -S.oz);
  const unsigned qnx = S.ix >= 0.f ? w1.x : w1.y, qfx = S.ix >= 0.f ? w1.y : w1.x;
  const unsigned qny = S.iy >= 0.f ? w1.z : w1.w, qfy = S.iy >= 0.f ? w1.w : w1.z;
  const unsigned qnz = S.iz >= 0.f ? w2.x : w2.y, qfz = S.iz >= 0.f ? w2.y : w2.x;
  rr[0] = (int)w2.z; rr[1] = (int)w2.w; rr[2] = (int)w3.x; rr[3] = (int)w3.y;
#define GVT_Q2(Q, SH) ((f2){ (float)(((Q) >> (SH)) & 0xffu), (float)(((Q) >> ((SH) + 8)) & 0xffu) })
#define GVT_SLAB2(SH, A, B)                                                                                          \
  {                                                                                                                  \
    const f2 nx_ = __builtin_elementwise_fma(GVT_Q2(qnx, SH), splat2(sx), splat2(bx.x));                              \
    const f2 ny_ = __builtin_elementwise_fma(GVT_Q2(qny, SH), splat2(sy), splat2(by.x));                              \
    const f2 nz_ = __builtin_elementwise_fma(GVT_Q2(qnz, SH), splat2(sz), splat2(bz.x));                              \
    const f2 fx_ = __builtin_elementwise_fma(GVT_Q2(qfx, SH), splat2(sx), splat2(bx.y));                              \
    const f2 fy_ = __builtin_elementwise_fma(GVT_Q2(qfy, SH), splat2(sy), splat2(by.y));                              \
    const f2 fz_ = __builtin_elementwise_fma(GVT_Q2(qfz, SH), splat2(sz), splat2(bz.y));                              \
    const float na_ = fmaxf(fmaxf(nx_.x, ny_.x), fmaxf(nz_.x, 0.f)), nb_ = fmaxf(fmaxf(nx_.y, ny_.y), fmaxf(nz_.y, 0.f)); \
    const float fa_ = fminf(fminf(fx_.x, fy_.x), fz_.x) * 1.0000004f, fb_ = fminf(fminf(fx_.y, fy_.y), fz_.y) * 1.0000004f; \
    const bool ha_ = na_ <= (LIM ? fminf(fa_, lim) : fa_), hb_ = nb_ <= (LIM ? fminf(fb_, lim) : fb_);                \
    tn[A] = ha_ ? na_ : GVT_FLT_MAX;                                                          \
    tn[B] = hb_ ? nb_ : GVT_FLT_MAX;                                                                                 \
    if (hit) { hit[A] = ha_; hit[B] = hb_; }                                                                         \
  }
  GVT_SLAB2(0, 0, 1) GVT_SLAB2(16, 2, 3)
#undef GVT_SLAB2
#undef GVT_Q2
}

__device__ __forceinline__ void sort4(float (&tn)[4], int (&rr)[4]) {
  auto ce = [&](int a, int b) {
    const bool sw = tn[b] < tn[a];
    const float ta = sw ? tn[b] : tn[a], tb = sw ? tn[a] : tn[b];
    const int ra = sw ? rr[b] : rr[a], rb = sw ? rr[a] : rr[b];
    tn[a] = ta; tn[b] = tb; rr[a] = ra; rr[b] = rb;
  };
  ce(0, 1); ce(2, 3); ce(0, 2); ce(1, 3); ce(1, 2);
}

__device__ __forceinline__ int *kt_spill_ptr(int *spill_base, int k) {
  unsigned t = threadIdx.x;
  asm volatile("" : "+v"(t));
  return spill_base + ((size_t)(blockIdx.x * TRAV_BLOCK + t) * TRAV_SPILL + (size_t)k);
}

__device__ inline int wave_find_seg(const WaveSet &W, unsigned g) {
  int lo = 0, hi = W.n_seg - 1;
  while (lo < hi) {
    const int mid = (lo + hi + 1) >> 1;
    if (W.segs[mid].begin <= g) lo = mid; else hi = mid - 1;
  }
  return lo;
}

__device__ inline void flush_pending(volatile unsigned *pend, int n_pend, const RayPlanes &q, const RayPlanes &out, unsigned *out_count, const TermSink &K,
                                     const int *__restrict__ ray_inst = nullptr, int *__restrict__ out_from = nullptr) {
  if (!K.fb) {
    unsigned base = 0;
    if (lane_id() == 0) base = atomicAdd(out_count, (unsigned)n_pend);
    base = (unsigned)__builtin_amdgcn_readfirstlane((int)base);
    for (int k = (int)lane_id(); k < n_pend; k += 64) {
      const unsigned src = pend[k];
      out.p0[base + k] = q.p0[src]; out.p1[base + k] = q.p1[src]; out.p2[base + k] = q.p2[src]; out.p3[base + k] = q.p3[src];
      if (out.p4) out.p4[base + k] = 0u;
      store_no_known(out, base + k);
      if (out_from) out_from[base + k] = ray_inst[src];
    }
    return;
  }
  const bool alone = K.top.n_inst == 1 && !ray_inst && K.from >= 0;
  for (int k0 = 0; k0 < n_pend; k0 += 64) {
    const int k = k0 + (int)lane_id();
    bool go_on = false;
    float4 a, b, c, d;
    int from = K.from;
    if (k < n_pend) {
      const unsigned src = pend[k];
      c = q.p2[src]; d = q.p3[src];
      if (!alone) {
        a = q.p0[src]; b = q.p1[src];
        if (ray_inst) from = ray_inst[src];
        float ret_t;
        go_on = top_nearest(a, b, K.top, from, ret_t) >= 0;
      }
      if (!go_on) deposit_shadow(K.fb, K.n_pix, __float_as_int(d.w), mk3(c.x, c.y, c.z), d.z, (unsigned)__float_as_int(d.x));
    }
    const unsigned long long m = ballot64(go_on);
    if (m) {
      unsigned base = 0;
      if (lane_id() == 0) base = atomicAdd(out_count, (unsigned)__popcll(m));
      base = (unsigned)__builtin_amdgcn_readfirstlane((int)base);
      if (go_on) { const unsigned slot = base + lanes_below(m); out.p0[slot] = a; out.p1[slot] = b; out.p2[slot] = c; out.p3[slot] = d; if (out.p4) out.p4[slot] = 0u; store_no_known(out, slot); if (out_from) out_from[slot] = from; }
    }
  }
}

template <unsigned frac8> __device__ __noinline__ uint3 kt_fetch(unsigned *counter, unsigned n, unsigned row, unsigned state) {
  const unsigned wpb = (unsigned)(TRAV_BLOCK / 64), n_waves_total = gridDim.x * wpb, share_w = n / n_waves_total;
  const unsigned chunk = max(64u, ((share_w * frac8 / 8u) + 16u) & ~31u), dyn = max(64u, (share_w / 16u) & ~63u);
  unsigned ub = 1u, ue = 0u;
  if (row == XCD_STRIPES_OFF) {
    unsigned base = 0, len = chunk;
    if (!(state & 16u)) base = (blockIdx.x * wpb + (threadIdx.x >> 6)) * chunk;
    else {
      if (lane_id() == 0) base = atomicAdd(counter, dyn);
      base = (unsigned)__builtin_amdgcn_readfirstlane((int)base) + n_waves_total * chunk;
      len = dyn;
    }
    if (base < n) { ub = base; ue = min(base + len, n); }
    return make_uint3(ub, ue, 16u);
  }
  const XcdStripeMap SM = xcd_stripe_map(n, dyn, row);
  const unsigned ks = max(1u, (chunk + dyn / 2u) / dyn), home = blockIdx.x & 7u;
  unsigned st_steal = state & 15u, st_left = (state & 16u) ? state >> 5 : ks;
  bool got = false;
  if (st_left) {
    const unsigned s = (blockIdx.x >> 3) * wpb + (threadIdx.x >> 6);
    got = xcd_stripe_unit(SM, home, s * ks + (ks - st_left), &ub, &ue);
    st_left = got ? st_left - 1u : 0u;
  }
  while (!got && st_steal < XCD_STRIPES) {
    const unsigned x = (home + st_steal) & 7u;
    unsigned t = 0;
    if (lane_id() == 0) t = atomicAdd(counter + cw_work_stripe(x), 1u);
    t = (unsigned)__builtin_amdgcn_readfirstlane((int)t) + ((gridDim.x + 7u - x) >> 3) * wpb * ks;
    got = xcd_stripe_unit(SM, x, t, &ub, &ue);
    if (!got) st_steal++;
  }
  if (!got) { ub = 1u; ue = 0u; }
  return make_uint3(ub, ue, st_steal | 16u | (st_left << 5));
}

#define KT_TAB 32
struct KtInst { Mat4 minv; const uint4 *nodes4; const float4 *tris; };
struct KtSeg { float4 *planes; unsigned long long cap; unsigned begin; int inst; };
struct MultiSrc {
  WaveSet W;
  int *ray_inst;
  int *out_from;
  unsigned long long *tot_any;
  const unsigned *cls_cnt;
  unsigned cls_stride;
  unsigned *cls_total;
  int *hop_inst;
  int hop_read;
  const int *hop_owner;
  int hop_rank;
  int hop_early;
  unsigned long long *hop_tot;
};
template <bool ANY, bool XFORM, int MODE, bool MULTI = false>
__global__ __launch_bounds__(TRAV_BLOCK, (ANY ? KT_BLOCKS_ANY : KT_BLOCKS_CLOSEST)) void k_trace(RayPlanes q, const unsigned *__restrict__ idx, unsigned n, Mat4 minv, Trav T, float tnear,
                                                       gvt_hip_hit *__restrict__ hits, int *__restrict__ flags, RayPlanes out, unsigned *out_count,
                                                       unsigned *counter, int *spill_base, int refill_min, int inner_min, const unsigned *__restrict__ n_dev, int share, unsigned share_min, TermSink sink, LongQ LQ,
                                                       MultiSrc MS = MultiSrc{}, unsigned stripe_row = XCD_STRIPES_OFF) {
  const unsigned n_waves_total = gridDim.x * (unsigned)(TRAV_BLOCK / 64);
  const float z12 = minv.m[3], z13 = minv.m[7], z14 = minv.m[11];
  if (n_dev) n = *n_dev;
  constexpr int N_CLS = (ANY && !MULTI) ? SHADOW_CLASSES : 0;
  __shared__ unsigned s_cls[N_CLS + 1];
  const bool by_class = N_CLS > 0 && MS.cls_cnt != nullptr;
  if (by_class) {
    if (threadIdx.x == 0) {
      unsigned acc = 0;
      for (int k = 0; k < N_CLS; k++) { s_cls[k] = acc; acc += MS.cls_cnt[N_CLS - 1 - k]; }
      s_cls[N_CLS] = acc;
      if (blockIdx.x == 0 && MS.cls_total) *MS.cls_total = acc;
    }
    __syncthreads();
    n = s_cls[N_CLS];
  }
  const unsigned share_w = n / n_waves_total;
  const unsigned chunk = max(64u, ((share_w * (ANY ? 5u : 3u) / 8u) + 16u) & ~31u);
  const unsigned dyn = max(64u, (share_w / 16u) & ~63u);
  __shared__ int stack[TRAV_STACK * TRAV_BLOCK];
  int *lds = &stack[threadIdx.x];
  int *spill_m = spill_base + (size_t)(blockIdx.x * TRAV_BLOCK + threadIdx.x) * TRAV_SPILL;
#define KT_SPILL(K) (*(MULTI ? spill_m + (K) : kt_spill_ptr(spill_base, (K))))
  __shared__ KtInst s_inst[MULTI ? KT_TAB : 1];
  __shared__ KtSeg s_seg[(MULTI && !ANY) ? KT_TAB : 1];
  bool tab = false;
  if (MULTI) {
    tab = MS.W.n_inst > 0 && MS.W.n_inst <= KT_TAB && MS.W.n_seg <= KT_TAB;
    if (tab) {
      for (int t = (int)threadIdx.x; t < MS.W.n_inst; t += TRAV_BLOCK) { const WaveInst *wi = MS.W.insts + t; s_inst[t].minv = wi->minv; s_inst[t].nodes4 = wi->nodes4; s_inst[t].tris = wi->tris; }
      if (!ANY)
        for (int t = TRAV_BLOCK - 1 - (int)threadIdx.x; t < MS.W.n_seg; t += TRAV_BLOCK) { const WaveSeg sg = MS.W.segs[t]; KtSeg k; k.planes = sg.planes; k.cap = sg.cap; k.begin = sg.begin; k.inst = sg.inst; s_seg[t] = k; }
      __syncthreads();
    }
  }
#define KT_PUSH(REF)                                                                  \
  {                                                                                   \
    if (sp < TRAV_STACK) { lds[sp * TRAV_BLOCK] = (REF); sp++; }                      \
    else if (sp - TRAV_STACK < TRAV_SPILL) { KT_SPILL(sp - TRAV_STACK) = (REF); sp++; }  \
    else atomicOr(counter + (CW_TRAV_OVF - CW_WORK), 1u);           \
  }
#define KT_POP()                                                                      \
  {                                                                                   \
    if (sp == sb) cur = TRAV_DONE;                                                    \
    else { sp--; if (sp < TRAV_STACK) cur = lds[sp * TRAV_BLOCK]; else cur = KT_SPILL(sp - TRAV_STACK); } \
  }
  __shared__ unsigned pend_all[(TRAV_BLOCK / 64) * 128];
  volatile unsigned *pend = &pend_all[(threadIdx.x >> 6) * 128];
  int n_pend = 0;
  unsigned c_next = 0, c_end = 0;
  bool exhausted = false;
  bool first_chunk = true;
  unsigned st_state = 0;
  bool active = false;
  unsigned j = 0;
  V3 O = mk3(0, 0, 0), D = mk3(0, 0, 1);
  RaySlab S = make_slab(0.f, 0.f, 0.f, 0.f, 0.f, 0.f);
  float bt = GVT_FLT_MAX, bu = 0.f, bv = 0.f, bden = 1.f;
  int bp = -1, sp = 0, cur = TRAV_DONE;
  int sb = 0;
  bool sharing = false;
  int drain_iters = 0;
  int nsteps = 0;
#define KT_PARKED (nsteps < 0)
  const uint4 *nodes4_l = T.nodes4;
  const float4 *tris_l = T.tris;
  int inst_l = 0;
  unsigned gidx = 0;
  unsigned n_started = 0;
  unsigned n_hops = 0;
#if GVT_STAMP
  unsigned long long st_refill = 0, st_inner = 0, st_leaf = 0, st_retire = 0, n_inner_it = 0, n_outer_it = 0, t_mark = 0, t_begin = __builtin_amdgcn_s_memtime();
  unsigned long long t_exh = 0, it_exh = 0, out_exh = 0, act_exh = 0, n_inner_lanes = 0, n_leaf_lanes = 0;
#endif
  for (;;) {
#if GVT_STAMP == 1
    { unsigned long long t_ = __builtin_amdgcn_s_memtime(); if (n_outer_it) st_retire += t_ - t_mark; t_mark = t_; }
#endif
    unsigned long long idle = ballot64(!active);
    int nidle = __popcll(idle);
    if (!exhausted && (nidle >= refill_min || nidle == 64)) {
      while (nidle > 0) {
        if (c_next == c_end) {
          if constexpr (!MULTI) {
            const uint3 f = kt_fetch<ANY ? 5u : 3u>(counter, n, stripe_row, st_state);
            const unsigned ub = (unsigned)__builtin_amdgcn_readfirstlane((int)f.x), ue = (unsigned)__builtin_amdgcn_readfirstlane((int)f.y);
            st_state = (unsigned)__builtin_amdgcn_readfirstlane((int)f.z);
            if (ub > ue) {
              exhausted = true;
#if GVT_STAMP
              if (!t_exh) { t_exh = __builtin_amdgcn_s_memtime(); it_exh = n_inner_it; out_exh = n_outer_it; act_exh = 64 - nidle; }
#endif
              break;
            }
            c_next = ub; c_end = ue;
            if (ub == ue) continue;
          } else {
          unsigned base = 0;
          unsigned this_chunk = chunk;
          if (first_chunk) {
            first_chunk = false;
            base = (blockIdx.x * (unsigned)(TRAV_BLOCK / 64) + (threadIdx.x >> 6)) * chunk;
          } else {
// ... 51 lines not shown
              O = xfm_point(s_inst[inst_l].minv, mk3(a.x, a.y, a.z)); D = xfm_vector(s_inst[inst_l].minv, mk3(b.x, b.y, b.z));
            } else if (start) {
              const WaveInst *wi = MS.W.insts + inst_l;
              nodes4_l = wi->nodes4; tris_l = wi->tris;
              O = xfm_point(wi->minv, mk3(a.x, a.y, a.z)); D = xfm_vector(wi->minv, mk3(b.x, b.y, b.z));
            }
          } else {
            a = q.p0[i]; b = q.p1[i];
            O = mk3(a.x, a.y, a.z); D = mk3(b.x, b.y, b.z);
            if (XFORM) {
              const float *m = minv.m;
              O = xfm_point(minv, O);
              D = mk3((m[0] * D.x + m[4] * D.y) + (m[8] * D.z + z12), (m[1] * D.x + m[5] * D.y) + (m[9] * D.z + z13), (m[2] * D.x + m[6] * D.y) + (m[10] * D.z + z14));
            }
            if (ANY && MODE >= 1) j = i;
          }
          if (start) {
            const float dx = fabsf(D.x) < 1e-30f ? copysignf(1e-30f, D.x) : D.x;
            const float dy = fabsf(D.y) < 1e-30f ? copysignf(1e-30f, D.y) : D.y;
            const float dz = fabsf(D.z) < 1e-30f ? copysignf(1e-30f, D.z) : D.z;
            const float ix = 1.0f / dx, iy = 1.0f / dy, iz = 1.0f / dz;
            S = make_slab(ix, iy, iz, O.x * ix, O.y * iy, O.z * iz);
            bt = GVT_FLT_MAX; bu = 0.f; bv = 0.f; bden = 1.f; bp = -1;
            sp = 0; sb = 0; nsteps = 0;
            cur = (MULTI ? nodes4_l : T.nodes4) != nullptr ? 0 : TRAV_DONE;
            active = true;
          }
        }
        if (MULTI && ANY) n_started += (unsigned)__popcll(ballot64(start));
        c_next += take;
        idle = ballot64(!active);
        nidle = __popcll(idle);
      }
    }
    if (nidle == 64) break;
    const bool share_on = ANY && (share & 1) != 0;
    if (exhausted) drain_iters++;
    const bool share_now = share_on && exhausted && drain_iters > KT_SHARE_DELAY && n >= share_min;
    if (share_now && nidle > 0) {
      unsigned long long idle_m = idle;
      unsigned long long don_m = ballot64(active && cur != TRAV_DONE && (sp - sb) >= 2);
      const unsigned wave_tid0 = threadIdx.x & ~63u;
      for (int pairs = 0; idle_m && don_m && pairs < 16; pairs++) {
        const int h = __ffsll((long long)idle_m) - 1, d = __ffsll((long long)don_m) - 1;
        const int sbd = __shfl(sb, d);
        const unsigned gj = (unsigned)__shfl((int)j, d);
        const float gOx = __shfl(O.x, d), gOy = __shfl(O.y, d), gOz = __shfl(O.z, d);
        const float gDx = __shfl(D.x, d), gDy = __shfl(D.y, d), gDz = __shfl(D.z, d);
        RaySlab gS;
        gS.ix = __shfl(S.ix, d); gS.iy = __shfl(S.iy, d); gS.iz = __shfl(S.iz, d);
        gS.ox = (f2){ __shfl(S.ox.x, d), __shfl(S.ox.y, d) }; gS.oy = (f2){ __shfl(S.oy.x, d), __shfl(S.oy.y, d) }; gS.oz = (f2){ __shfl(S.oz.x, d), __shfl(S.oz.y, d) };
        const int gbp = __shfl(bp, d);
        const int ginst = __shfl(inst_l, d);
        if ((int)lane_id() == h) {
          if (MULTI) { inst_l = ginst; nodes4_l = MS.W.insts[ginst].nodes4; tris_l = MS.W.insts[ginst].tris; }
          const unsigned tid_d = wave_tid0 + (unsigned)d;
          cur = (sbd < TRAV_STACK) ? stack[sbd * TRAV_BLOCK + tid_d]
                                   : spill_base[((size_t)blockIdx.x * TRAV_BLOCK + tid_d) * TRAV_SPILL + (sbd - TRAV_STACK)];
          j = gj; O = mk3(gOx, gOy, gOz); D = mk3(gDx, gDy, gDz);
          S = gS; bp = gbp;
          sp = 0; sb = 0;
          active = true;
        }
        if ((int)lane_id() == d) sb++;
        idle_m &= idle_m - 1;
        don_m &= don_m - 1;
        sharing = true;
#if GVT_STAMP
        if (lane_id() == 0) atomicAdd(&g_stamp[23], 1ull);
#endif
      }
    }
#if GVT_STAMP == 1
    { unsigned long long t_ = __builtin_amdgcn_s_memtime(); st_refill += t_ - t_mark; t_mark = t_; n_outer_it++; }
#endif
    unsigned long long im = ballot64(cur >= 0);
    const float lim2 = fminf(cull_bound(bt), 3.40282326e38f);
    while (im) {
      const bool at_inner = cur >= 0;
      if (at_inner) {
        float tn[4];
        int rr[4];
        bool entered[4];
        node4_test<ANY>((const uint4 *)((const char *)(MULTI ? nodes4_l : T.nodes4) + ((unsigned)cur << 6)), S, GVT_FLT_MAX, tn, rr, ANY ? entered : nullptr);
#define KT_ENTERED(K) (ANY ? entered[K] : (tn[K] <= lim2))
        if (!ANY) sort4(tn, rr);
        int nxt = TRAV_DONE;
        bool have = false;
        if (sp + 3 <= TRAV_STACK) {
#pragma unroll
          for (int c4 = 3; c4 >= 0; c4--) {
            if (KT_ENTERED(c4)) {
              if (have) { lds[sp * TRAV_BLOCK] = nxt; sp++; }
              nxt = rr[c4]; have = true;
            }
          }
        } else {
#pragma unroll
          for (int c4 = 3; c4 >= 0; c4--) {
            if (KT_ENTERED(c4)) {
              if (have) KT_PUSH(nxt)
              nxt = rr[c4]; have = true;
            }
          }
        }
        if (have) cur = nxt;
        else KT_POP()
#undef KT_ENTERED
      }
#if GVT_STAMP == 1
      n_inner_it++; n_inner_lanes += (unsigned long long)__popcll(ballot64(at_inner));
#endif
      if (!ANY && at_inner && LQ.steps && ++nsteps > (exhausted ? LQ.steps_drain : LQ.steps) && cur != TRAV_DONE) { KT_PUSH(cur) cur = TRAV_DONE; nsteps = -1; }
      im = ballot64(cur >= 0);
      if (__popcll(im) < inner_min) break;
    }
#if GVT_STAMP == 1
    { unsigned long long t_ = __builtin_amdgcn_s_memtime(); st_inner += t_ - t_mark; t_mark = t_; }
#endif
    {
      const bool at_leaf = cur < 0 && cur != TRAV_DONE;
#if GVT_STAMP == 1
      n_leaf_lanes += (unsigned long long)__popcll(ballot64(at_leaf));
#endif
      if (at_leaf) {
        const unsigned code = (unsigned)~cur;
        const unsigned first = code >> 3, ntri = code & 7u;
        const float4 *ts = (MULTI ? tris_l : T.tris) + 4 * (size_t)first;
        bool occluded = false;
        for (unsigned kb = 0; kb < ntri && !(ANY && occluded); kb += 2) {
          float4 s0[2], s1[2], s2[2];
#pragma unroll
          for (unsigned k = 0; k < 2; k++)
            if (kb + k < ntri) { s0[k] = ts[4 * (kb + k)]; s1[k] = ts[4 * (kb + k) + 1]; s2[k] = ts[4 * (kb + k) + 2]; }
#pragma unroll
          for (unsigned k = 0; k < 2; k++) {
            if (kb + k < ntri && !(ANY && occluded)) {
              const V3 e1 = mk3(s1[k].x, s1[k].y, s1[k].z), e2 = mk3(s2[k].x, s2[k].y, s2[k].z);
              float TT, U, V, aden;
              if (tri_test_raw(O, D, mk3(s0[k].x, s0[k].y, s0[k].z), e1, e2, cross3(e1, e2), tnear, TT, U, V, aden)) {
                const float t = TT / aden;
                if (t <= GVT_FLT_MAX) {
                  if (ANY) occluded = true;
                  else {
                    const int prim = __float_as_int(s0[k].w);
                    if (bp < 0 || t < bt || (t == bt && prim < bp)) { bt = t; bp = prim; bu = U; bv = V; bden = aden; }
                  }
                }
              }
            }
          }
        }
        if (ANY && occluded) bp = 0;
      }
      if (at_leaf) {
        if (ANY && bp == 0) cur = TRAV_DONE;
        else KT_POP()
      }
    }
#if GVT_STAMP == 1
    { unsigned long long t_ = __builtin_amdgcn_s_memtime(); st_leaf += t_ - t_mark; t_mark = t_; }
#endif
    {
      const int nfin_w = __popcll(ballot64(active && cur == TRAV_DONE)), nidle_w = __popcll(ballot64(!active));
      const bool retire_now = RETIRE_BATCH == 0 || share_now || nfin_w + nidle_w >= (exhausted ? 64 : refill_min);
      if (!retire_now) continue;
    }
    if (sharing) {
      const unsigned long long FM = ballot64(active && cur == TRAV_DONE);
      unsigned long long fm = FM;
      while (fm) {
        const int f = __ffsll((long long)fm) - 1;
        const unsigned jf = (unsigned)__shfl((int)j, f);
        const unsigned long long G = ballot64(active && j == jf);
        const unsigned long long Gf = G & FM, A = G & ~FM;
        const int tgt = A ? __ffsll((long long)A) - 1 : __ffsll((long long)Gf) - 1;
        unsigned long long src = Gf & ~(1ull << tgt);
        bool merged_occluded = false;
        while (src) {
          const int sidx = __ffsll((long long)src) - 1;
          if (__shfl(bp, sidx) >= 0) merged_occluded = true;
          if ((int)lane_id() == sidx) active = false;
          src &= src - 1;
        }
        if (merged_occluded && ((G >> lane_id()) & 1ull) && active) { bp = 0; cur = TRAV_DONE; }
        fm &= ~Gf;
      }
    }
    if (MULTI && (ANY ? (MODE == 1 && MS.hop_tot != nullptr) : (MS.hop_inst != nullptr))) {
      const bool cand = active && cur == TRAV_DONE && bp < 0 && (ANY || !KT_PARKED) && !(exhausted && MS.hop_early);
      if (ballot64(cand)) {
        bool hopped = false;
        if (cand) {
          float4 *slot0;
          float4 a, b;
          if (ANY) { slot0 = q.p0 + j; b = q.p1[j]; }
          else {
            const WaveSeg sg = MS.W.segs[wave_find_seg(MS.W, gidx)];
            const unsigned local = gidx - sg.begin;
            slot0 = sg.planes + local; b = sg.planes[sg.cap + local];
          }
          a = *slot0;
          float ret_t;
          const int next = top_nearest(a, b, sink.top, inst_l, ret_t);
          if (next >= 0 && (!MS.hop_owner || MS.hop_owner[next] == MS.hop_rank)) {
            const V3 o = add3(mk3(a.x, a.y, a.z), scl3(mk3(b.x, b.y, b.z), ret_t * 0.95f));
            a.x = o.x; a.y = o.y; a.z = o.z;
            *slot0 = a;
            if (ANY) MS.ray_inst[j] = next; else MS.hop_inst[gidx] = next;
            inst_l = next;
            const WaveInst *wi = MS.W.insts + next;
            nodes4_l = wi->nodes4; tris_l = wi->tris;
            O = xfm_point(wi->minv, o); D = xfm_vector(wi->minv, mk3(b.x, b.y, b.z));
            const float dx = fabsf(D.x) < 1e-30f ? copysignf(1e-30f, D.x) : D.x;
            const float dy = fabsf(D.y) < 1e-30f ? copysignf(1e-30f, D.y) : D.y;
            const float dz = fabsf(D.z) < 1e-30f ? copysignf(1e-30f, D.z) : D.z;
            const float ix = 1.0f / dx, iy = 1.0f / dy, iz = 1.0f / dz;
            S = make_slab(ix, iy, iz, O.x * ix, O.y * iy, O.z * iz);
            bt = GVT_FLT_MAX; bu = 0.f; bv = 0.f; bden = 1.f; bp = -1;
            sp = 0; sb = 0; nsteps = 0;
            cur = nodes4_l != nullptr ? 0 : TRAV_DONE;
            hopped = true;
          }
        }
        n_hops += (unsigned)__popcll(ballot64(hopped));
      }
    }
    const bool fin = active && cur == TRAV_DONE;
    if (ANY && MODE == 1) {
      const bool survive = fin && bp < 0;
      const unsigned long long sm = ballot64(survive);
      if (sm) {
        if (survive) pend[n_pend + lanes_below(sm)] = j;
        n_pend += __popcll(sm);
      }
      if (n_pend >= 64) { flush_pending(pend, n_pend, q, out, out_count, sink, MULTI ? MS.ray_inst : nullptr, MULTI ? MS.out_from : nullptr); n_pend = 0; }
    }
    if (!ANY && LQ.steps) {
      const unsigned long long pm = ballot64(fin && KT_PARKED);
      if (pm) {
        unsigned base = 0;
        if ((int)lane_id() == __ffsll((long long)pm) - 1) base = atomicAdd(LQ.count, (unsigned)__popcll(pm));
        base = __shfl(base, __ffsll((long long)pm) - 1);
        if (fin && KT_PARKED) {
          const unsigned slot = base + lanes_below(pm);
          LongRec R; R.j = j; R.i = MULTI ? gidx : (idx ? idx[j] : j); R.bt = bt; R.bp = bp; R.bu = bu; R.bv = bv; R.bden = bden; R.ns = 0u;
          const int depth = sp - sb;
          if (LQ.stk && depth > 0 && depth <= LONG_SAVE && slot < LQ.stk_cap) {
            int *dst = LQ.stk + (size_t)slot * LONG_SAVE;
            for (int k = 0; k < depth; k++) dst[k] = (sb + k < TRAV_STACK) ? lds[(sb + k) * TRAV_BLOCK] : KT_SPILL(sb + k - TRAV_STACK);
            R.ns = (unsigned)depth;
          }
          LQ.recs[slot] = R;
        }
      }
    }
    if (ANY && MODE == 2) {
      if (fin && bp >= 0) {
        const unsigned px = ((const unsigned *)q.p2)[j];
        if (px != 0xffffffffu) ((float4 *)sink.fb)[px] = make_float4(0.f, 0.f, 0.f, 0.f);
      }
    }
    if (fin) {
      if (ANY) { if (MODE == 0) flags[j] = (bp >= 0) ? 1 : 0; }
      else {
        if (!KT_PARKED) { gvt_hip_hit h; h.t = bt; h.prim = bp; h.u = (bp >= 0) ? bu / bden : 0.f; h.v = (bp >= 0) ? bv / bden : 0.f; hits[j] = h; }
        if (LQ.steps_out) LQ.steps_out[j] = (unsigned char)(KT_PARKED ? 255 : min(nsteps, 254));
      }
      active = false;
    }
  }
#if GVT_STAMP
  if (lane_id() == 0) { atomicAdd(&g_stamp[0], st_refill); atomicAdd(&g_stamp[1], st_inner); atomicAdd(&g_stamp[2], st_leaf); atomicAdd(&g_stamp[3], st_retire); atomicAdd(&g_stamp[4], n_inner_it); atomicAdd(&g_stamp[5], n_outer_it); atomicAdd(&g_stamp[6], 1ull); atomicAdd(&g_stamp[7], (unsigned long long)__builtin_amdgcn_s_memtime() - t_begin); atomicAdd(&g_stamp[14], n_inner_lanes); atomicAdd(&g_stamp[15], n_leaf_lanes); atomicMax(&g_stamp[16], ~t_begin); atomicMax(&g_stamp[17], (unsigned long long)__builtin_amdgcn_s_memtime()); atomicMax(&g_stamp[18], t_exh); atomicAdd(&g_stamp[19], t_exh ? t_exh - t_begin : 0ull); atomicMax(&g_stamp[20], (unsigned long long)__builtin_amdgcn_s_memtime() - t_begin); atomicMax(&g_stamp[21], t_exh ? t_exh - t_begin : 0ull); atomicMax(&g_stamp[22], ~(t_exh ? t_exh - t_begin : ~0ull));
    if (t_exh) { atomicAdd(&g_stamp[8], (unsigned long long)__builtin_amdgcn_s_memtime() - t_exh); atomicAdd(&g_stamp[9], n_inner_it - it_exh); atomicAdd(&g_stamp[10], n_outer_it - out_exh); atomicAdd(&g_stamp[11], act_exh); atomicMax(&g_stamp[12], (unsigned long long)__builtin_amdgcn_s_memtime() - t_exh); atomicMax(&g_stamp[13], n_inner_it - it_exh); } }
#endif
  if (ANY && MODE == 1) { if (n_pend) flush_pending(pend, n_pend, q, out, out_count, sink, MULTI ? MS.ray_inst : nullptr, MULTI ? MS.out_from : nullptr); }
  if (MULTI && ANY && MS.tot_any && n_started && lane_id() == 0) atomicAdd(MS.tot_any, (unsigned long long)n_started);
  if (MULTI && MS.hop_tot && n_hops && lane_id() == 0) atomicAdd(MS.hop_tot, (unsigned long long)n_hops);
#undef KT_PUSH
#undef KT_POP
#undef KT_SPILL
#undef KT_PARKED
}
```

### gravit_amd/csrc/trace_wave.inc

```
#define LONG_CAP 512
#define LONG_PHYS (LONG_CAP + 256)

struct WaveLists { volatile int *s_ref; volatile float *s_tn; volatile int *l_ref; volatile float *l_tn; };

__device__ __forceinline__ bool within_best(float etn, float bt) { return etn <= cull_bound(bt); }
__device__ __forceinline__ bool closer(float t, int p, float bt, int bp) { return bp < 0 || t < bt || (t == bt && p < bp); }

#define CL_GROUPS 12
template <bool CLUSTER>
struct WaveFan {
  static constexpr int OPEN = CLUSTER ? CL_GROUPS : 64;
  static constexpr int NODES = CLUSTER ? 16 : 3;
  static constexpr int LEAVES = CLUSTER ? 20 : 4;
};

template <bool ANY, bool CLUSTER>
__device__ __forceinline__ void wave_nodes(const uint4 *__restrict__ nodes, const RaySlab &S, const WaveLists &L, int take, int &ns, int &nl, float bt) {
  const int lane = (int)lane_id();
  const int g = CLUSTER ? lane / 5 : lane, role = CLUSTER ? lane - 5 * g : 0;
  const bool mine = g < take;
  int ent = 0;
  float etn = 0.f;
  if (mine) { ent = L.s_ref[ns - 1 - g]; if constexpr (!ANY) etn = L.s_tn[ns - 1 - g]; }
  __builtin_amdgcn_wave_barrier();
  ns -= take;
  bool act = mine && (ANY || within_best(etn, bt));
  const uint4 *nd;
  if constexpr (CLUSTER) {
    const unsigned mask = (unsigned)ent & 15u;
    act = act && (role == 0 || ((mask >> (role - 1)) & 1u));
    const unsigned slot = ((unsigned)ent >> 4) + (role ? 1u + (unsigned)__popc(mask & ((1u << (role - 1)) - 1u)) : 0u);
    nd = nodes + (size_t)GVT_NODE4_F4 * slot;
  } else nd = nodes + (size_t)GVT_NODE4_F4 * ent;
  float tn[4];
  int rr[4];
  bool entered[4] = { false, false, false, false };
  auto in = [&](int c) { return ANY ? entered[c] : tn[c] < GVT_FLT_MAX; };
  unsigned verdict = 0u;
  if (act) {
    if constexpr (ANY) node4_test(nd, S, GVT_FLT_MAX, tn, rr, entered);
    else node4_test(nd, S, bt, tn, rr);
    if (CLUSTER && role == 0) verdict = (in(0) ? 1u : 0u) | (in(1) ? 2u : 0u) | (in(2) ? 4u : 0u) | (in(3) ? 8u : 0u);
    if constexpr (!ANY) sort4(tn, rr);
  }
  bool open = act;
  if constexpr (CLUSTER) {
    const unsigned pv = (unsigned)__shfl((int)verdict, 5 * g);
    open = act && (role == 0 || ((pv >> (role - 1)) & 1u));
  }
#pragma unroll
  for (int c = 3; c >= 0; c--) {
    const bool hit = open && in(c);
    const bool inner = hit && rr[c] >= 0 && !(CLUSTER && role == 0), leaf = hit && rr[c] < 0;
    const unsigned long long mi = ballot64(inner), ml = ballot64(leaf);
    if (inner) { const int pos = ns + (int)lanes_below(mi); L.s_ref[pos] = rr[c]; if constexpr (!ANY) L.s_tn[pos] = tn[c]; }
    if (leaf) { const int pos = nl + (int)lanes_below(ml); L.l_ref[pos] = rr[c]; if constexpr (!ANY) L.l_tn[pos] = tn[c]; }
    ns += __popcll(mi);
    nl += __popcll(ml);
  }
  __builtin_amdgcn_wave_barrier();
}

template <bool ANY>
__device__ __forceinline__ bool wave_leaves(const float4 *__restrict__ tris, V3 O, V3 D, float tnear, const WaveLists &L, int &nl,
                                            float &bt, int &bp, float &bu, float &bv, float &bden) {
  const int lane = (int)lane_id();
  const int take = min(nl, 64);
  const bool mine = lane < take;
  int ref = -1;
  float etn = 0.f;
  if (mine) { ref = L.l_ref[nl - 1 - lane]; if constexpr (!ANY) etn = L.l_tn[nl - 1 - lane]; }
  __builtin_amdgcn_wave_barrier();
  nl -= take;
  float lt = GVT_FLT_MAX, lu = 0.f, lv = 0.f, ld = 1.f;
  int lp = -1;
  bool hit_any = false;
  if (mine && (ANY || within_best(etn, bt))) {
    const unsigned code = (unsigned)~ref;
    const unsigned first = code >> 3, ntri = code & 7u;
    const float4 *ts = tris + 4 * (size_t)first;
    for (unsigned k = 0; k < ntri && !hit_any; k++) {
      const float4 s0 = ts[4 * k], s1 = ts[4 * k + 1], s2 = ts[4 * k + 2];
      const V3 e1 = mk3(s1.x, s1.y, s1.z), e2 = mk3(s2.x, s2.y, s2.z);
      float TT, U, V, aden;
      if (tri_test_raw(O, D, mk3(s0.x, s0.y, s0.z), e1, e2, cross3(e1, e2), tnear, TT, U, V, aden)) {
        const float t = TT / aden;
        if (t <= GVT_FLT_MAX) {
          if constexpr (ANY) hit_any = true;
          else {
            const int prim = __float_as_int(s0.w);
            if (closer(t, prim, lt, lp)) { lt = t; lp = prim; lu = U; lv = V; ld = aden; }
          }
        }
      }
    }
  }
  if constexpr (ANY) return ballot64(hit_any) != 0ull;
  if (ballot64(lp >= 0)) {
#pragma unroll
    for (int off = 32; off >= 1; off >>= 1) {
      const float ot = __shfl_xor(lt, off), ou = __shfl_xor(lu, off), ov = __shfl_xor(lv, off), od = __shfl_xor(ld, off);
      const int op = __shfl_xor(lp, off);
      if (op >= 0 && closer(ot, op, lt, lp)) { lt = ot; lp = op; lu = ou; lv = ov; ld = od; }
    }
    if (lp >= 0 && closer(lt, lp, bt, bp)) { bt = lt; bp = lp; bu = lu; bv = lv; bden = ld; }
  }
  return false;
}

template <bool ANY, bool CLUSTER, int CAP, int PHYS>
__device__ __forceinline__ bool wave_run(const uint4 *__restrict__ nodes, const float4 *__restrict__ tris, V3 O, V3 D, const RaySlab &S, float tnear, const WaveLists &L,
                                          int ns, int nl, float &bt, int &bp, float &bu, float &bv, float &bden, unsigned *ovf_word) {
  using F = WaveFan<CLUSTER>;
  const int lane = (int)lane_id();
  bool occluded = false;
  while (!occluded && (ns > 0 || nl > 0)) {
    const bool do_leaf = nl > 0 && (ns == 0 || nl >= 64 || nl > CAP - 256);
    if (!do_leaf) {
      int take = min(min(ns, F::OPEN), min((CAP - ns) / F::NODES, (CAP - nl) / F::LEAVES));
      take = max(take, 1);
      if (ns + F::NODES * take > PHYS || nl + F::LEAVES * take > PHYS) { if (lane == 0) atomicOr(ovf_word, 1u); break; }
      wave_nodes<ANY, CLUSTER>(nodes, S, L, take, ns, nl, bt);
    } else occluded = wave_leaves<ANY>(tris, O, D, tnear, L, nl, bt, bp, bu, bv, bden);
  }
  return occluded;
}
template <bool CLUSTER, int CAP, int PHYS>
__device__ __forceinline__ bool wave_any_run(const uint4 *__restrict__ nodes, int root_entry, const float4 *__restrict__ tris, V3 O, V3 D, const RaySlab &S, float tnear,
                                              volatile int *s_ref, volatile int *l_ref, unsigned *ovf_word) {
  if (lane_id() == 0) s_ref[0] = CLUSTER ? root_entry : 0;
  __builtin_amdgcn_wave_barrier();
  float bt = GVT_FLT_MAX, bu = 0.f, bv = 0.f, bden = 1.f;
  int bp = -1;
  return wave_run<true, CLUSTER, CAP, PHYS>(nodes, tris, O, D, S, tnear, WaveLists{ s_ref, nullptr, l_ref, nullptr }, (CLUSTER || nodes) ? 1 : 0, 0, bt, bp, bu, bv, bden, ovf_word);
}
__device__ __forceinline__ RaySlab slab_of(V3 O, V3 D) {
  const float dx = fabsf(D.x) < 1e-30f ? copysignf(1e-30f, D.x) : D.x;
  const float dy = fabsf(D.y) < 1e-30f ? copysignf(1e-30f, D.y) : D.y;
  const float dz = fabsf(D.z) < 1e-30f ? copysignf(1e-30f, D.z) : D.z;
  const float ix = 1.0f / dx, iy = 1.0f / dy, iz = 1.0f / dz;
  return make_slab(ix, iy, iz, O.x * ix, O.y * iy, O.z * iz);
}

__device__ __forceinline__ unsigned wave_ticket(bool &first, unsigned *counter, int wv) {
  if (first) { first = false; return blockIdx.x * 4u + (unsigned)wv; }
  unsigned r = 0;
  if (lane_id() == 0) r = atomicAdd(counter, 1u);
  return (unsigned)__builtin_amdgcn_readfirstlane((int)r) + gridDim.x * 4u;
}

template <bool XFORM, bool MULTI = false>
__global__ __launch_bounds__(256) void k_long_closest(RayPlanes q, const LongRec *__restrict__ recs, const unsigned *__restrict__ n_recs, Mat4 minv,
                                                       Trav T, float tnear, gvt_hip_hit *__restrict__ hits, unsigned *counter, WaveSet W = WaveSet{},
                                                       const int *__restrict__ stk = nullptr, const int *__restrict__ hop_inst = nullptr) {
  __shared__ int s_ref_all[4][LONG_PHYS];
  __shared__ float s_tn_all[4][LONG_PHYS];
  __shared__ int l_ref_all[4][LONG_PHYS];
  __shared__ float l_tn_all[4][LONG_PHYS];
  const int wv = threadIdx.x >> 6;
  const int lane = (int)lane_id();
  volatile int *s_ref = s_ref_all[wv];
  volatile float *s_tn = s_tn_all[wv];
  volatile int *l_ref = l_ref_all[wv];
  volatile float *l_tn = l_tn_all[wv];
  const unsigned n = *n_recs;
  bool first = true;
  for (;;) {
    const unsigned r = wave_ticket(first, counter, wv);
    if (r >= n) break;
    const LongRec R = recs[r];
    float4 a, b;
    V3 O, D;
    if (MULTI) {
      const WaveSeg sg = W.segs[wave_find_seg(W, R.i)];
      const unsigned local = R.i - sg.begin;
      a = sg.planes[local]; b = sg.planes[sg.cap + local];
      int inst = sg.inst;
      if (hop_inst) { const int h_ = hop_inst[R.i]; if (h_ >= 0) inst = h_; }
      const WaveInst *wi = W.insts + inst;
      T.nodes4 = wi->nodes4; T.tris = wi->tris;
      O = xfm_point(wi->minv, mk3(a.x, a.y, a.z)); D = xfm_vector(wi->minv, mk3(b.x, b.y, b.z));
    } else {
      a = q.p0[R.i]; b = q.p1[R.i];
      O = mk3(a.x, a.y, a.z); D = mk3(b.x, b.y, b.z);
      if (XFORM) { O = xfm_point(minv, O); D = xfm_vector(minv, D); }
    }
    const RaySlab S = slab_of(O, D);
    float bt = R.bt, bu = R.bu, bv = R.bv, bden = R.bden;
    int bp = R.bp;
    int ns = T.nodes4 ? 1 : 0, nl = 0;
    if (stk && R.ns && T.nodes4) {
      const int e = lane < (int)R.ns ? stk[(size_t)r * LONG_SAVE + lane] : TRAV_DONE;
      const bool is_node = lane < (int)R.ns && e >= 0, is_leaf = lane < (int)R.ns && e < 0 && e != TRAV_DONE;
      const unsigned long long mi = ballot64(is_node), ml = ballot64(is_leaf);
      if (is_node) { s_ref[lanes_below(mi)] = e; s_tn[lanes_below(mi)] = 0.f; }
      if (is_leaf) { l_ref[lanes_below(ml)] = e; l_tn[lanes_below(ml)] = 0.f; }
      ns = __popcll(mi); nl = __popcll(ml);
    } else if (lane == 0) { s_ref[0] = 0; s_tn[0] = 0.f; }
    __builtin_amdgcn_wave_barrier();
    wave_run<false, false, LONG_CAP, LONG_PHYS>(T.nodes4, T.tris, O, D, S, tnear, WaveLists{ s_ref, s_tn, l_ref, l_tn }, ns, nl, bt, bp, bu, bv, bden, counter + (CW_TRAV_OVF - CW_LONG_WORK));
    { gvt_hip_hit h; h.t = bt; h.prim = bp; h.u = (bp >= 0) ? bu / bden : 0.f; h.v = (bp >= 0) ? bv / bden : 0.f; hits[R.j] = h; }
  }
}

__global__ __launch_bounds__(256) void k_long_seed(LongRec *__restrict__ recs, unsigned *__restrict__ count, const unsigned *__restrict__ idx, unsigned n,
                                                    const unsigned *__restrict__ n_dev) {
  if (n_dev) n = *n_dev;
  const unsigned j = blockIdx.x * blockDim.x + threadIdx.x;
  if (j == 0) *count = n;
  if (j >= n) return;
  LongRec R; R.j = j; R.i = idx ? idx[j] : j; R.bt = GVT_FLT_MAX; R.bp = -1; R.bu = 0.f; R.bv = 0.f; R.bden = 1.f; R.ns = 0u;
  recs[j] = R;
}

template <bool MULTI>
__global__ __launch_bounds__(256) void k_wave_any(RayPlanes q, const unsigned *__restrict__ n_dev, Mat4 minv, Trav T, float tnear, RayPlanes out,
                                                   unsigned *out_count, unsigned *counter, TermSink sink, MultiSrc MS) {
  __shared__ int s_ref_all[4][LONG_PHYS];
  __shared__ int l_ref_all[4][LONG_PHYS];
  const int wv = threadIdx.x >> 6;
  const int lane = (int)lane_id();
  volatile int *s_ref = s_ref_all[wv];
  volatile int *l_ref = l_ref_all[wv];
  const unsigned n = *n_dev;
  bool first = true;
  for (;;) {
    const unsigned r = wave_ticket(first, counter, wv);
    if (r >= n) break;
    const float4 a = q.p0[r], b = q.p1[r];
    int inst = sink.from;
    V3 O, D;
    if (MULTI) {
      inst = MS.ray_inst[r];
      const WaveInst *wi = MS.W.insts + inst;
      T.nodes4 = wi->nodes4; T.tris = wi->tris;
      O = xfm_point(wi->minv, mk3(a.x, a.y, a.z)); D = xfm_vector(wi->minv, mk3(b.x, b.y, b.z));
    } else {
      O = xfm_point(minv, mk3(a.x, a.y, a.z)); D = xfm_vector(minv, mk3(b.x, b.y, b.z));
    }
    const bool occluded = wave_any_run<false, LONG_CAP, LONG_PHYS>(T.nodes4, 0, T.tris, O, D, slab_of(O, D), tnear, s_ref, l_ref, counter + (CW_TRAV_OVF - CW_WORK));
    if (!occluded && lane == 0) {
      const float4 c = q.p2[r], d = q.p3[r];
      bool go_on = true;
      if (sink.fb) {
        float ret_t;
        go_on = top_nearest(a, b, sink.top, inst, ret_t) >= 0;
        if (!go_on) deposit_shadow(sink.fb, sink.n_pix, __float_as_int(d.w), mk3(c.x, c.y, c.z), d.z, (unsigned)__float_as_int(d.x));
      }
      if (go_on) {
        const unsigned slot = atomicAdd(out_count, 1u);
        out.p0[slot] = a; out.p1[slot] = b; out.p2[slot] = c; out.p3[slot] = d;
        if (out.p4) out.p4[slot] = 0u;
        store_no_known(out, slot);
        if (MULTI && MS.out_from) MS.out_from[slot] = inst;
      }
    }
    __builtin_amdgcn_wave_barrier();
  }
}
```

### include/gvt_hip.h

```cpp
#ifndef GVT_HIP_H
#define GVT_HIP_H

#include <stddef.h>
#include <stdint.h>

#ifdef __cplusplus
extern "C" {
#endif

#define GVT_HIP_ABI_VERSION 6
int gvt_hip_abi_version(void);

#define GVT_HIP_OK 0
#define GVT_HIP_ERR_INVALID (-1)
#define GVT_HIP_ERR_DEVICE (-2)
#define GVT_HIP_ERR_CAPACITY (-3)
#define GVT_HIP_ERR_NODEVICE (-4)
#define GVT_HIP_ERR_TIMEOUT (-5)
#define GVT_HIP_ERR_PEER (-6)

#define GVT_HIP_NORMALS_FLAT 0
#define GVT_HIP_NORMALS_SMOOTH 1

typedef struct gvt_hip_ray {
// ... 93 lines not shown
int gvt_hip_queue_reserve(gvt_hip_queue *, size_t capacity);
int gvt_hip_queue_clear(gvt_hip_queue *);
int gvt_hip_queue_size(gvt_hip_queue *, size_t *n);
#define GVT_HIP_APPEND_DEVICE 1
#define GVT_HIP_APPEND_KEEP_STATE 2
int gvt_hip_queue_append_flags(gvt_hip_queue *, const gvt_hip_ray *rays, size_t n, int flags);
int gvt_hip_queue_append(gvt_hip_queue *, const gvt_hip_ray *rays, size_t n, int src_on_device);
int gvt_hip_queue_export(gvt_hip_queue *, gvt_hip_ray *dst, size_t cap, size_t *n, int dst_on_device);
int gvt_hip_trace_queue(gvt_hip_mesh *, gvt_hip_queue *q_in, gvt_hip_queue *q_out, const float m[16], const float minv[16],
                        const float normi[9], const gvt_hip_light *lights, size_t n_lights, int normal_mode, uint32_t seed);
int gvt_hip_trace_queue_sink(gvt_hip_mesh *, gvt_hip_queue *q, gvt_hip_queue *moved, const float m[16], const float minv[16],
                             const float normi[9], const gvt_hip_light *lights, size_t n_lights, int normal_mode, uint32_t seed,
                             gvt_hip_top *top, int from_inst, gvt_hip_fb *fb);

int gvt_hip_camera_generate(gvt_hip_queue *q, const float eye[3], const float focus[3], const float up[3], float fov,
                            int width, int height, int samples, int depth, float jitter_window_size);
int gvt_hip_camera_generate_tiled(gvt_hip_queue *q, const float eye[3], const float focus[3], const float up[3], float fov,
                                  int width, int height, int samples, int depth, float jitter_window_size, int tile);

gvt_hip_top *gvt_hip_top_create(const float *inst_lo, const float *inst_hi, size_t n_inst);
void gvt_hip_top_destroy(gvt_hip_top *);
int gvt_hip_top_order(const gvt_hip_top *, int32_t *order_out );
int gvt_hip_top_update(gvt_hip_top *, const float *inst_lo, const float *inst_hi, size_t n_inst);
int gvt_hip_shuffle(gvt_hip_top *, gvt_hip_queue *q_in, int from, gvt_hip_queue *const *queues ,
                    const uint8_t *keep_mask, gvt_hip_fb *fb);
int gvt_hip_queue_sizes(gvt_hip_queue *const *queues, size_t n, uint64_t *sizes_out);

typedef struct gvt_hip_camera {
  float eye[3], focus[3], up[3];
  float fov;
  int32_t width, height, samples, depth;
  float jitter_window_size;
} gvt_hip_camera;
int gvt_hip_camera_filter(gvt_hip_top *, const gvt_hip_camera *cam, int tile, gvt_hip_queue *const *queues, const uint8_t *keep_mask);
int gvt_hip_image_frame(gvt_hip_top *, gvt_hip_mesh *const *meshes, const float *m , const float *minv, const float *normi ,
                        size_t n_inst, const gvt_hip_light *lights, size_t n_lights, int normal_mode, const gvt_hip_camera *cam,
                        gvt_hip_queue *const *queues, gvt_hip_queue *q_cam, gvt_hip_queue *q_moved, gvt_hip_fb *fb, uint64_t *adapter_calls);

typedef struct gvt_hip_comm gvt_hip_comm;
typedef struct gvt_hip_hub gvt_hip_hub;
typedef struct gvt_hip_tracer gvt_hip_tracer;
int gvt_hip_comm_unique_id(unsigned char id[128]);
gvt_hip_comm *gvt_hip_comm_create(const unsigned char id[128], int rank, int world);
gvt_hip_hub *gvt_hip_hub_create(int world);
void gvt_hip_hub_abort(gvt_hip_hub *);
void gvt_hip_hub_destroy(gvt_hip_hub *);
gvt_hip_comm *gvt_hip_comm_create_local(gvt_hip_hub *, int rank);
void gvt_hip_comm_destroy(gvt_hip_comm *);
int gvt_hip_comm_selftest(gvt_hip_comm *, size_t bytes);
int gvt_hip_comm_rank(const gvt_hip_comm *);
int gvt_hip_comm_count(const gvt_hip_comm *);
int gvt_hip_comm_reserved_cus(const gvt_hip_comm *);
int gvt_hip_comm_set_deadline_ms(gvt_hip_comm *, int ms);
int gvt_hip_comm_world(const gvt_hip_comm *);

gvt_hip_tracer *gvt_hip_tracer_create(gvt_hip_top *, gvt_hip_mesh *const *meshes, const float *m , const float *minv,
                                      const float *normi , size_t n_inst, const gvt_hip_light *lights, size_t n_lights,
                                      int normal_mode, const gvt_hip_camera *cam, gvt_hip_fb *fb);
void gvt_hip_tracer_destroy(gvt_hip_tracer *);
int gvt_hip_tracer_set_camera(gvt_hip_tracer *, const gvt_hip_camera *cam);
int gvt_hip_tracer_set_transforms(gvt_hip_tracer *, const float *m , const float *minv, const float *normi , size_t n_inst);
int gvt_hip_tracer_set_domains(gvt_hip_tracer *, const int32_t *owner , gvt_hip_comm *comm);
#define GVT_HIP_FRAME_BSP 1
#define GVT_HIP_FRAME_NO_COMPOSITE 2
#define GVT_HIP_FRAME_IMAGE 8
#define GVT_HIP_FRAME_FULL_REDUCE 4
typedef struct gvt_hip_frame_stats {
  uint64_t rounds;
  uint64_t chains;
  uint64_t host_syncs;
  uint64_t rays_sent;
  uint64_t rays_closest;
  uint64_t rays_any;
  uint64_t packets_bailed;
  uint64_t bytes_sent;
  double ms_chain;
  double ms_announce;
  double ms_payload;
  double ms_composite;
  double ms_host_wait;
  uint64_t exchanges;
  uint64_t rays_inline;
  uint64_t early_deposit_launches;
} gvt_hip_frame_stats;
int gvt_hip_tracer_frame(gvt_hip_tracer *, int flags, gvt_hip_frame_stats *stats);

#define GVT_HIP_RAY_OPAQUE 0x2
#define GVT_HIP_RAY_BOUNDARY 0x4
#define GVT_HIP_RAY_EXTERNAL_BOUNDARY 0x10
#define GVT_HIP_VOLUME_OPAQUE_A 0.99f
#define GVT_HIP_VOLUME_DEVICE 1
#define GVT_HIP_VOLUME_NO_SKIP 2
typedef struct gvt_hip_volume gvt_hip_volume;
gvt_hip_volume *gvt_hip_volume_create(const float *samples, const int counts[3], const float origin[3], const float spacing[3], const int offset[3],
                                      const int global_counts[3], float sampling_rate, int flags);
void gvt_hip_volume_destroy(gvt_hip_volume *);
typedef struct gvt_hip_volume_info {
  float box_lo[3], box_hi[3];
  float dt;
  float value_min, value_max;
  int32_t blocks[3];
  float pad;
  uint64_t n_blocks, n_blocks_empty;
  uint64_t samples_marched;
  uint64_t samples_gathered;
} gvt_hip_volume_info;
int gvt_hip_volume_get_info(gvt_hip_volume *, gvt_hip_volume_info *);
int gvt_hip_volume_update_samples(gvt_hip_volume *, const float *samples, size_t n_samples, uint32_t flags, float *ms_out );
#define GVT_HIP_VOXEL_F32 0
#define GVT_HIP_VOXEL_U8 1
#define GVT_HIP_VOXEL_I16 2
#define GVT_HIP_VOXEL_U16 3
gvt_hip_volume *gvt_hip_volume_create_typed(const void *samples, int voxel_type, const int counts[3], const float origin[3], const float spacing[3],
                                            const int offset[3], const int global_counts[3], float sampling_rate, int flags);
int gvt_hip_volume_update_samples_typed(gvt_hip_volume *, const void *samples, int voxel_type, size_t n_samples, uint32_t flags, float *ms_out );
int gvt_hip_volume_get_voxel_type(gvt_hip_volume *, int *type_out, size_t *sample_bytes_out);
int gvt_hip_volume_set_transfer(gvt_hip_volume *, const float *cmap, int nc, const float *omap, int no, float value_lo, float value_hi);
int gvt_hip_volume_trace(gvt_hip_volume *, const gvt_hip_ray *rays, size_t n, size_t begin, size_t end, gvt_hip_ray *rays_out, size_t cap,
                         size_t *n_out, const float m[16], const float minv[16]);
int gvt_hip_shuffle_volume(gvt_hip_top *, gvt_hip_queue *q_in, int from, gvt_hip_queue *const *queues, gvt_hip_fb *fb);
int gvt_hip_volume_frame(gvt_hip_top *, gvt_hip_volume *const *volumes, const float *m , const float *minv, size_t n_inst,
                         const gvt_hip_camera *cam, gvt_hip_queue *const *queues, gvt_hip_fb *fb, uint64_t *adapter_calls);

#define GVT_HIP_RAY_SIDES 0x20
#define GVT_HIP_VOLUME_MAX_SURFACES 16
#define GVT_HIP_VOLUME_MAX_LIGHTS 8
int gvt_hip_volume_set_surfaces(gvt_hip_volume *, const float *isovalues, int n_iso, const float *slices , int n_slices, float opacity);
int gvt_hip_volume_set_lights(gvt_hip_volume *, const float *positions , const float *colours , int n, float ka, float kd);
int gvt_hip_volume_get_crossings(gvt_hip_volume *, uint64_t *crossings_rendered);

#define GVT_HIP_VOLUME_SHADE_NONE 0
#define GVT_HIP_VOLUME_SHADE_GRADIENT 1
int gvt_hip_volume_set_shading(gvt_hip_volume *, int mode);
int gvt_hip_volume_get_shading(gvt_hip_volume *, int *mode_out);
int gvt_hip_volume_get_shaded(gvt_hip_volume *, uint64_t *samples_shaded);

#define GVT_HIP_VOLUME_GRADIENT_CELL 0
#define GVT_HIP_VOLUME_GRADIENT_CENTRAL 1
int gvt_hip_volume_set_ghosts(gvt_hip_volume *, const void *const faces[6], int voxel_type, uint32_t flags);
int gvt_hip_volume_set_gradient(gvt_hip_volume *, int kind);
int gvt_hip_volume_get_gradient(gvt_hip_volume *, int *kind_out, uint64_t *central_marches_out);

#define GVT_HIP_RAY_CLIP 0x40
typedef struct gvt_hip_depth gvt_hip_depth;
gvt_hip_depth *gvt_hip_depth_create(int width, int height);
void gvt_hip_depth_destroy(gvt_hip_depth *);
int gvt_hip_depth_clear(gvt_hip_depth *);
int gvt_hip_depth_upload(gvt_hip_depth *, const float *t , uint32_t flags);
int gvt_hip_depth_download(gvt_hip_depth *, float *t );
int gvt_hip_depth_render(gvt_hip_depth *, gvt_hip_mesh *const *meshes, const float *m , const float *minv, size_t n_inst,
                         const gvt_hip_camera *cam);
int gvt_hip_volume_frame_clipped(gvt_hip_top *, gvt_hip_volume *const *volumes, const float *m , const float *minv, size_t n_inst,
                                 const gvt_hip_camera *cam, gvt_hip_queue *const *queues, gvt_hip_fb *fb, const gvt_hip_depth *depth,
                                 uint64_t *adapter_calls);
int gvt_hip_fb_composite_over(gvt_hip_fb *front, const gvt_hip_fb *back, const gvt_hip_depth *depth);

#define GVT_HIP_VOLUME_AMR_SHADED 8
#define GVT_HIP_VOLUME_MAX_SUBGRIDS 4096
#define GVT_HIP_VOLUME_MAX_LEVELS 4
typedef struct gvt_hip_subgrid {
  int32_t parent;
  int32_t ratio;
  int32_t lo[3];
  int32_t cells[3];
} gvt_hip_subgrid;
int gvt_hip_volume_set_subgrids(gvt_hip_volume *, const gvt_hip_subgrid *grids, const float *const *samples, int n, int flags);
// ... 170 lines not shown
```

Before: 2509 Mrays/s.

## Store flat geometric normal in hit record to skip shade-time triangle fetch

```diff
diff --git a/gravit_amd/capi.py b/gravit_amd/capi.py
--- a/gravit_amd/capi.py
+++ b/gravit_amd/capi.py
@@ -66,7 +66,8 @@
     _fields_ = [("rounds", C.c_uint64), ("chains", C.c_uint64), ("host_syncs", C.c_uint64), ("rays_sent", C.c_uint64),
                 ("rays_closest", C.c_uint64), ("rays_any", C.c_uint64), ("packets_bailed", C.c_uint64), ("bytes_sent", C.c_uint64),
                 ("ms_chain", C.c_double), ("ms_announce", C.c_double), ("ms_payload", C.c_double), ("ms_composite", C.c_double), ("ms_host_wait", C.c_double),
-                ("exchanges", C.c_uint64), ("rays_inline", C.c_uint64), ("early_deposit_launches", C.c_uint64)]
+                ("exchanges", C.c_uint64), ("rays_inline", C.c_uint64), ("early_deposit_launches", C.c_uint64),
+                ("normal_record_launches", C.c_uint64)]
 
     def as_dict(self):
         return {k: getattr(self, k) for k, _ in self._fields_}
diff --git a/gravit_amd/csrc/api.hip b/gravit_amd/csrc/api.hip
--- a/gravit_amd/csrc/api.hip
+++ b/gravit_amd/csrc/api.hip
@@ -240,6 +240,7 @@
   { "packet_min_rays", &Knobs::packet_min_rays, 0, 1 << 30, true },
   { "shadow_order", &Knobs::shadow_order, 0, 1, true },       { "shadow_order_min_rays", &Knobs::shadow_order_min_rays, 0, 1 << 30, true },
   { "xcd_stripes", &Knobs::xcd_stripes, 0, 1, true },           { "early_deposit", &Knobs::early_deposit, 0, 1, true },
+  { "normal_records", &Knobs::normal_records, 0, 1, true },
 
   { "inline_kb", &Knobs::inline_kb, 0, 1024, true },          { "comm_cus", &Knobs::comm_cus, 0, 128, true },
   { "comm_stream", &Knobs::comm_stream, 0, 1, true },         { "spec_ticks", &Knobs::spec_ticks, 0, 1, true },
diff --git a/gravit_amd/csrc/domain.hip b/gravit_amd/csrc/domain.hip
--- a/gravit_amd/csrc/domain.hip
+++ b/gravit_amd/csrc/domain.hip
@@ -1295,7 +1295,7 @@
   R->cam_row_rays = 0u;
   bool first_on_device = false;
   R->fb_fresh = true;
-  const uint64_t early0 = C.early_deposit_launches;
+  const uint64_t early0 = C.early_deposit_launches, nrec0 = C.normal_record_launches;
   if (!lean) {
     if ((rc = gvt_hip_fb_clear(R->fb))) return rc;
     k_zero_totals<<<(unsigned)std::max<size_t>(1, (nI + 255) / 256), 256, 0, st>>>(C.d_counters, R->d_overflow, R->fb->w, R->fb->h, R->d_count_ptr, (int)nI);
@@ -1624,6 +1624,7 @@
   }
   R->frame_no++;
   S.early_deposit_launches = C.early_deposit_launches - early0;
+  S.normal_record_launches = C.normal_record_launches - nrec0;
   if (out) *out = S;
   return 0;
 }
diff --git a/gravit_amd/csrc/gvt_device.h b/gravit_amd/csrc/gvt_device.h
--- a/gravit_amd/csrc/gvt_device.h
+++ b/gravit_amd/csrc/gvt_device.h
@@ -44,22 +44,7 @@
 static_assert(CW_SHADOW_CLS + 8 <= CW_WORK_XCD && CW_PEEK <= CW_WORK_XCD, "no named counter word shares a line with the counters of stripes 1..7 (stripe 0 keeps CW_WORK's)");
 static_assert(CW_LONG_WORK == 4 && CW_BOUNCE_A < 5 && CW_LONG < 5, "k_trace_begin / launch_closest zero words 0..4 as one run");
 
-struct V3 {
-  float x, y, z;
-};
-__host__ __device__ inline V3 mk3(float x, float y, float z) { V3 r; r.x = x; r.y = y; r.z = z; return r; }
-__host__ __device__ inline V3 ld3(const float *p) { return mk3(p[0], p[1], p[2]); }
-__host__ __device__ inline V3 add3(V3 a, V3 b) { return mk3(a.x + b.x, a.y + b.y, a.z + b.z); }
-__host__ __device__ inline V3 sub3(V3 a, V3 b) { return mk3(a.x - b.x, a.y - b.y, a.z - b.z); }
-__host__ __device__ inline V3 mul3(V3 a, V3 b) { return mk3(a.x * b.x, a.y * b.y, a.z * b.z); }
-__host__ __device__ inline V3 scl3(V3 a, float s) { return mk3(a.x * s, a.y * s, a.z * s); }
-__host__ __device__ inline V3 neg3(V3 a) { return mk3(-a.x, -a.y, -a.z); }
-__host__ __device__ inline float dot3(V3 a, V3 b) { V3 t = mul3(a, b); return t.x + t.y + t.z; }
-__host__ __device__ inline V3 cross3(V3 x, V3 y) {
-  return mk3(x.y * y.z - y.y * x.z, x.z * y.x - y.z * x.x, x.x * y.y - y.x * x.y);
-}
-__host__ __device__ inline float len3(V3 a) { return sqrtf(dot3(a, a)); }
-__host__ __device__ inline V3 norm3(V3 a) { return scl3(a, 1.0f / sqrtf(dot3(a, a))); }
+#include "gvt_vec3.h"
 
 struct Mat4 {
   float m[16];
diff --git a/gravit_amd/csrc/gvt_internal.h b/gravit_amd/csrc/gvt_internal.h
--- a/gravit_amd/csrc/gvt_internal.h
+++ b/gravit_amd/csrc/gvt_internal.h
@@ -67,6 +67,7 @@
   int shadow_cls_lo = 24, shadow_cls_shift = 3;
   int xcd_stripes = 1;
   int early_deposit = 1;
+  int normal_records = 1;
   int shadow_order_min_rays = 262144;
   int packet_min_rays = 524288;
   int packet_sah_max = 128;
@@ -113,6 +114,7 @@
   gvt_hip_stats stats{};
   int n_cu = 256;
   uint64_t early_deposit_launches = 0;
+  uint64_t normal_record_launches = 0;
   bool shadow_order_denied = false;
   int cu_reserved = 0;
   int trav_blocks = 0;
diff --git a/gravit_amd/csrc/gvt_vec3.h b/gravit_amd/csrc/gvt_vec3.h
--- /dev/null
+++ b/gravit_amd/csrc/gvt_vec3.h
@@ -0,0 +1,25 @@
+#pragma once
+#include <math.h>
+#if !defined(__HIPCC__) && !defined(__host__)
+#define __host__
+#define __device__
+#endif
+
+struct V3 {
+  float x, y, z;
+};
+__host__ __device__ inline V3 mk3(float x, float y, float z) { V3 r; r.x = x; r.y = y; r.z = z; return r; }
+__host__ __device__ inline V3 ld3(const float *p) { return mk3(p[0], p[1], p[2]); }
+__host__ __device__ inline V3 add3(V3 a, V3 b) { return mk3(a.x + b.x, a.y + b.y, a.z + b.z); }
+__host__ __device__ inline V3 sub3(V3 a, V3 b) { return mk3(a.x - b.x, a.y - b.y, a.z - b.z); }
+__host__ __device__ inline V3 mul3(V3 a, V3 b) { return mk3(a.x * b.x, a.y * b.y, a.z * b.z); }
+__host__ __device__ inline V3 scl3(V3 a, float s) { return mk3(a.x * s, a.y * s, a.z * s); }
+__host__ __device__ inline V3 neg3(V3 a) { return mk3(-a.x, -a.y, -a.z); }
+__host__ __device__ inline float dot3(V3 a, V3 b) { V3 t = mul3(a, b); return t.x + t.y + t.z; }
+__host__ __device__ inline V3 cross3(V3 x, V3 y) {
+  return mk3(x.y * y.z - y.y * x.z, x.z * y.x - y.z * x.x, x.x * y.y - y.x * x.y);
+}
+__host__ __device__ inline float len3(V3 a) { return sqrtf(dot3(a, a)); }
+__host__ __device__ inline V3 norm3(V3 a) { return scl3(a, 1.0f / sqrtf(dot3(a, a))); }
+
+__host__ __device__ inline V3 flat_neg_ng(V3 e1, V3 e2) { return cross3(sub3(mk3(0.f, 0.f, 0.f), e1), e2); }
diff --git a/gravit_amd/csrc/shade.inc b/gravit_amd/csrc/shade.inc
--- a/gravit_amd/csrc/shade.inc
+++ b/gravit_amd/csrc/shade.inc
@@ -170,6 +170,7 @@
   unsigned cls_stride;
   int cls_lo, cls_shift;
   int early_deposit;
+  int normal_records;
 };
 
 __device__ __forceinline__ void store_shadow_early(const ShadeArgs &A, unsigned slot, const RayRec &s) {
@@ -232,18 +233,23 @@
     r = load_ray(in, i);
     h = A.hits[j];
     if (!LEAN) g_seed = (A.first_pass && (!A.carried_rng || r.rng == 0u)) ? ray_stream_seed(A.seed, A.index_base + gi) : r.rng;
-    if (h.prim < 0) {
+    const bool nrec = LEAN && !MULTI && A.normal_records;
+    if (nrec ? h.t < 0.f : h.prim < 0) {
       miss = true;
     } else if (r.type != 1) {
       shaded = true;
       float t = h.t;
       r.t = t;
-      const float4 *sl = M->slots + 4 * (size_t)M->slot_of[h.prim];
-      const float4 s0 = sl[0], s1 = sl[1], s2 = sl[2], s3 = sl[3];
-      const V3 v0 = mk3(s0.x, s0.y, s0.z), v1 = mk3(s1.w, s2.w, s3.x), v2 = mk3(s3.y, s3.z, s3.w);
+      V3 negNg;
       int ia = 0, ib = 0, ic = 0;
-      if (A.normal_mode == GVT_HIP_NORMALS_SMOOTH || (!LEAN && M->vcolors)) { ia = M->tris[3 * h.prim]; ib = M->tris[3 * h.prim + 1]; ic = M->tris[3 * h.prim + 2]; }
-      const V3 negNg = cross3(sub3(v1, v0), sub3(v2, v0));
+      if (nrec) negNg = mk3(__int_as_float(h.prim), h.u, h.v);
+      else {
+        const float4 *sl = M->slots + 4 * (size_t)M->slot_of[h.prim];
+        const float4 s0 = sl[0], s1 = sl[1], s2 = sl[2], s3 = sl[3];
+        const V3 v0 = mk3(s0.x, s0.y, s0.z), v1 = mk3(s1.w, s2.w, s3.x), v2 = mk3(s3.y, s3.z, s3.w);
+        if (A.normal_mode == GVT_HIP_NORMALS_SMOOTH || (!LEAN && M->vcolors)) { ia = M->tris[3 * h.prim]; ib = M->tris[3 * h.prim + 1]; ic = M->tris[3 * h.prim + 2]; }
+        negNg = cross3(sub3(v1, v0), sub3(v2, v0));
+      }
       const V3 normalflat = norm3(mat3_mul(normi, negNg));
       if (A.normal_mode == GVT_HIP_NORMALS_SMOOTH) {
         const V3 a = ld3(M->normals + 3 * ib), b = ld3(M->normals + 3 * ic), c = ld3(M->normals + 3 * ia);
diff --git a/gravit_amd/csrc/trace.hip b/gravit_amd/csrc/trace.hip
--- a/gravit_amd/csrc/trace.hip
+++ b/gravit_amd/csrc/trace.hip
@@ -209,12 +209,27 @@
 
 template <bool XFORM, bool MULTI>
 static void closest_step(StepMode mode, const TraceSrc &S, const unsigned *idx, size_t n, const unsigned *n_dev, float tnear, gvt_hip_hit *d_hits, const LongQ &LQ,
-                         LongRec *d_long, bool later_pass = false) {
+                         LongRec *d_long, bool later_pass = false, bool normal_records = false) {
   Ctx &C = gctx();
   hipStream_t st = C.stream;
   unsigned *c = C.d_counters;
   const int tail_grid = C.n_cu * 3;
   RayPlanes none{};
+  if constexpr (XFORM && !MULTI) {
+    if (normal_records && mode == BY_LANES) {
+      {
+        ProfScope ps(KC_CLOSEST);
+        launch_trace<false, true, 1, false>(trav_grid2(n, true), st, S.q, idx, (unsigned)n, S.minv, S.T, tnear, d_hits, nullptr, none, nullptr, c + CW_WORK, C.d_spill,
+                                            C.refill_min, C.inner_min, n_dev, C.share, (unsigned)C.share_min_rays, S.sink, LQ, S.MS, stripe_arg(S.row));
+      }
+      if (LQ.steps) {
+        ProfScope ps(KC_LONG);
+        k_long_closest<true, false, true><<<tail_grid, 256, 0, st>>>(S.q, LQ.recs, LQ.count, S.minv, S.T, tnear, d_hits, c + CW_LONG_WORK, S.W, LQ.stk, S.hop);
+      }
+      C.normal_record_launches++;
+      return;
+    }
+  }
   if (mode == BY_PACKETS) {
     ProfScope ps(KC_CLOSEST);
     LongQ LP{ d_long, c + CW_LONG, nullptr, 0u, 0, 0 };
@@ -490,14 +505,16 @@
   const bool small1 = K.small && have4;
   const bool pkt = walks_packets(C, M, n) && W1.coherent && p.pass == 0 && have4 && !small1;
   const bool pkt_any = pkt && C.packet == 2;
-  closest_step<true, false>(pkt ? BY_PACKETS : small1 ? BY_WAVES : BY_LANES, S, p.idx, n, p.n_dev, GVT_RAY_EPSILON, K.B.hits, LQ, K.d_long);
+  const bool lean_shade = W1.coherent && p.pass == 0 && K.passes == 1 && K.P.sink.fb && K.P.sink.top.n_inst == 1 && nL >= 1 && plain_lambert(M) && no_area_light(K.lights_host, nL);
+  const bool normal_records = lean_shade && K.P.normal_mode == GVT_HIP_NORMALS_FLAT && !pkt && !small1 && C.normal_records;
+  closest_step<true, false>(pkt ? BY_PACKETS : small1 ? BY_WAVES : BY_LANES, S, p.idx, n, p.n_dev, GVT_RAY_EPSILON, K.B.hits, LQ, K.d_long, false, normal_records);
   ShadeArgs A = shade_args(K.B, p.idx, n, p.pass, p.n_dev, p.next, p.c_next, K.outp, K.out->d_count, K.P);
   A.in = W1.planes; A.normi = W1.normi; A.sink.from = W1.inst;
   if (pkt_any) { A.shadow_inst = K.d_shadow_inst; A.shadow_stride = (unsigned)n; }
   A.steps = K.B.steps; A.cls_cnt = by_class ? c + CW_SHADOW_CLS : nullptr; A.cls_stride = (unsigned)cls_stride; A.cls_lo = C.shadow_cls_lo; A.cls_shift = C.shadow_cls_shift;
-  const bool lean_shade = W1.coherent && p.pass == 0 && K.passes == 1 && K.P.sink.fb && K.P.sink.top.n_inst == 1 && nL >= 1 && plain_lambert(M) && no_area_light(K.lights_host, nL);
   const bool early_deposit = lean_shade && nL == 1 && K.P.one_writer && !small1 && !pkt_any && C.early_deposit;
   A.early_deposit = early_deposit ? 1 : 0;
+  A.normal_records = normal_records ? 1 : 0;
   shade_step<false>(A, mesh_view(M), lean_shade);
   if (!nL) return 0;
   TraceSrc SA = S;
diff --git a/gravit_amd/csrc/trace_lane.inc b/gravit_amd/csrc/trace_lane.inc
--- a/gravit_amd/csrc/trace_lane.inc
+++ b/gravit_amd/csrc/trace_lane.inc
@@ -41,9 +41,9 @@
   return S;
 }
 __device__ __forceinline__ f2 splat2(float v) { return (f2){ v, v }; }
-template <bool LIM = true>
+template <bool LIM = true, bool NOLIM = false>
 __device__ __forceinline__ void node4_test(const uint4 *__restrict__ nd, const RaySlab &S, float lim, float tn[4], int rr[4], bool *hit = nullptr) {
-  if (LIM) lim = cull_bound(lim);
+  if (LIM && !NOLIM) lim = cull_bound(lim);
   const uint4 w0 = nd[0], w1 = nd[1], w2 = nd[2], w3 = nd[3];
   const float sx = __uint_as_float(w0.w) * S.ix, sy = __uint_as_float(w3.z) * S.iy, sz = __uint_as_float(w3.w) * S.iz;
   const f2 bx = __builtin_elementwise_fma(splat2(__uint_as_float(w0.x)), splat2(S.ix), -S.ox);
@@ -64,7 +64,8 @@
     const f2 fz_ = __builtin_elementwise_fma(GVT_Q2(qfz, SH), splat2(sz), splat2(bz.y));                              \
     const float na_ = fmaxf(fmaxf(nx_.x, ny_.x), fmaxf(nz_.x, 0.f)), nb_ = fmaxf(fmaxf(nx_.y, ny_.y), fmaxf(nz_.y, 0.f)); \
     const float fa_ = fminf(fminf(fx_.x, fy_.x), fz_.x) * 1.0000004f, fb_ = fminf(fminf(fx_.y, fy_.y), fz_.y) * 1.0000004f; \
-    const bool ha_ = na_ <= (LIM ? fminf(fa_, lim) : fa_), hb_ = nb_ <= (LIM ? fminf(fb_, lim) : fb_);                \
+    const bool ha_ = NOLIM ? !(na_ > fa_) : na_ <= (LIM ? fminf(fa_, lim) : fa_);                                    \
+    const bool hb_ = NOLIM ? !(nb_ > fb_) : nb_ <= (LIM ? fminf(fb_, lim) : fb_);                                    \
     tn[A] = ha_ ? na_ : GVT_FLT_MAX;                                                          \
     tn[B] = hb_ ? nb_ : GVT_FLT_MAX;                                                                                 \
     if (hit) { hit[A] = ha_; hit[B] = hb_; }                                                                         \
@@ -200,6 +201,7 @@
                                                        gvt_hip_hit *__restrict__ hits, int *__restrict__ flags, RayPlanes out, unsigned *out_count,
                                                        unsigned *counter, int *spill_base, int refill_min, int inner_min, const unsigned *__restrict__ n_dev, int share, unsigned share_min, TermSink sink, LongQ LQ,
                                                        MultiSrc MS = MultiSrc{}, unsigned stripe_row = XCD_STRIPES_OFF) {
+  constexpr bool NREC = !ANY && !MULTI && MODE == 1;
   const unsigned n_waves_total = gridDim.x * (unsigned)(TRAV_BLOCK / 64);
   const float z12 = minv.m[3], z13 = minv.m[7], z14 = minv.m[11];
   if (n_dev) n = *n_dev;
@@ -220,6 +222,8 @@
   const unsigned chunk = max(64u, ((share_w * (ANY ? 5u : 3u) / 8u) + 16u) & ~31u);
   const unsigned dyn = max(64u, (share_w / 16u) & ~63u);
   __shared__ int stack[TRAV_STACK * TRAV_BLOCK];
+  __shared__ float s_nrm[NREC ? 3 * TRAV_BLOCK : 1];
+  float *nrm = &s_nrm[NREC ? threadIdx.x : 0];
   int *lds = &stack[threadIdx.x];
   int *spill_m = spill_base + (size_t)(blockIdx.x * TRAV_BLOCK + threadIdx.x) * TRAV_SPILL;
 #define KT_SPILL(K) (*(MULTI ? spill_m + (K) : kt_spill_ptr(spill_base, (K))))
@@ -437,7 +441,7 @@
         float tn[4];
         int rr[4];
         bool entered[4];
-        node4_test<ANY>((const uint4 *)((const char *)(MULTI ? nodes4_l : T.nodes4) + ((unsigned)cur << 6)), S, GVT_FLT_MAX, tn, rr, ANY ? entered : nullptr);
+        node4_test<ANY, ANY>((const uint4 *)((const char *)(MULTI ? nodes4_l : T.nodes4) + ((unsigned)cur << 6)), S, GVT_FLT_MAX, tn, rr, ANY ? entered : nullptr);
 #define KT_ENTERED(K) (ANY ? entered[K] : (tn[K] <= lim2))
         if (!ANY) sort4(tn, rr);
         int nxt = TRAV_DONE;
@@ -499,7 +503,11 @@
                   if (ANY) occluded = true;
                   else {
                     const int prim = __float_as_int(s0[k].w);
-                    if (bp < 0 || t < bt || (t == bt && prim < bp)) { bt = t; bp = prim; bu = U; bv = V; bden = aden; }
+                    if (bp < 0 || t < bt || (t == bt && prim < bp)) {
+                      bt = t; bp = prim;
+                      if (NREC) { const V3 n_ = flat_neg_ng(e1, e2); nrm[0] = n_.x; nrm[TRAV_BLOCK] = n_.y; nrm[2 * TRAV_BLOCK] = n_.z; }
+                      else { bu = U; bv = V; bden = aden; }
+                    }
                   }
                 }
               }
@@ -600,6 +608,7 @@
         if (fin && KT_PARKED) {
           const unsigned slot = base + lanes_below(pm);
           LongRec R; R.j = j; R.i = MULTI ? gidx : (idx ? idx[j] : j); R.bt = bt; R.bp = bp; R.bu = bu; R.bv = bv; R.bden = bden; R.ns = 0u;
+          if (NREC && bp >= 0) { R.bu = nrm[0]; R.bv = nrm[TRAV_BLOCK]; R.bden = nrm[2 * TRAV_BLOCK]; }
           const int depth = sp - sb;
           if (LQ.stk && depth > 0 && depth <= LONG_SAVE && slot < LQ.stk_cap) {
             int *dst = LQ.stk + (size_t)slot * LONG_SAVE;
@@ -619,7 +628,8 @@
     if (fin) {
       if (ANY) { if (MODE == 0) flags[j] = (bp >= 0) ? 1 : 0; }
       else {
-        if (!KT_PARKED) { gvt_hip_hit h; h.t = bt; h.prim = bp; h.u = (bp >= 0) ? bu / bden : 0.f; h.v = (bp >= 0) ? bv / bden : 0.f; hits[j] = h; }
+        if (NREC) { if (!KT_PARKED) ((float4 *)hits)[j] = bp >= 0 ? make_float4(bt, nrm[0], nrm[TRAV_BLOCK], nrm[2 * TRAV_BLOCK]) : make_float4(-1.0f, 0.f, 0.f, 0.f); }
+        else if (!KT_PARKED) { gvt_hip_hit h; h.t = bt; h.prim = bp; h.u = (bp >= 0) ? bu / bden : 0.f; h.v = (bp >= 0) ? bv / bden : 0.f; hits[j] = h; }
         if (LQ.steps_out) LQ.steps_out[j] = (unsigned char)(KT_PARKED ? 255 : min(nsteps, 254));
       }
       active = false;
diff --git a/gravit_amd/csrc/trace_wave.inc b/gravit_amd/csrc/trace_wave.inc
--- a/gravit_amd/csrc/trace_wave.inc
+++ b/gravit_amd/csrc/trace_wave.inc
@@ -38,7 +38,7 @@
   auto in = [&](int c) { return ANY ? entered[c] : tn[c] < GVT_FLT_MAX; };
   unsigned verdict = 0u;
   if (act) {
-    if constexpr (ANY) node4_test(nd, S, GVT_FLT_MAX, tn, rr, entered);
+    if constexpr (ANY) node4_test<true, true>(nd, S, GVT_FLT_MAX, tn, rr, entered);
     else node4_test(nd, S, bt, tn, rr);
     if (CLUSTER && role == 0) verdict = (in(0) ? 1u : 0u) | (in(1) ? 2u : 0u) | (in(2) ? 4u : 0u) | (in(3) ? 8u : 0u);
     if constexpr (!ANY) sort4(tn, rr);
@@ -61,7 +61,7 @@
   __builtin_amdgcn_wave_barrier();
 }
 
-template <bool ANY>
+template <bool ANY, bool NREC = false>
 __device__ __forceinline__ bool wave_leaves(const float4 *__restrict__ tris, V3 O, V3 D, float tnear, const WaveLists &L, int &nl,
                                             float &bt, int &bp, float &bu, float &bv, float &bden) {
   const int lane = (int)lane_id();
@@ -89,7 +89,11 @@
           if constexpr (ANY) hit_any = true;
           else {
             const int prim = __float_as_int(s0.w);
-            if (closer(t, prim, lt, lp)) { lt = t; lp = prim; lu = U; lv = V; ld = aden; }
+            if (closer(t, prim, lt, lp)) {
+              lt = t; lp = prim;
+              if constexpr (NREC) { const V3 n_ = flat_neg_ng(e1, e2); lu = n_.x; lv = n_.y; ld = n_.z; }
+              else { lu = U; lv = V; ld = aden; }
+            }
           }
         }
       }
@@ -108,7 +112,7 @@
   return false;
 }
 
-template <bool ANY, bool CLUSTER, int CAP, int PHYS>
+template <bool ANY, bool CLUSTER, int CAP, int PHYS, bool NREC = false>
 __device__ __forceinline__ bool wave_run(const uint4 *__restrict__ nodes, const float4 *__restrict__ tris, V3 O, V3 D, const RaySlab &S, float tnear, const WaveLists &L,
                                           int ns, int nl, float &bt, int &bp, float &bu, float &bv, float &bden, unsigned *ovf_word) {
   using F = WaveFan<CLUSTER>;
@@ -121,7 +125,7 @@
       take = max(take, 1);
       if (ns + F::NODES * take > PHYS || nl + F::LEAVES * take > PHYS) { if (lane == 0) atomicOr(ovf_word, 1u); break; }
       wave_nodes<ANY, CLUSTER>(nodes, S, L, take, ns, nl, bt);
-    } else occluded = wave_leaves<ANY>(tris, O, D, tnear, L, nl, bt, bp, bu, bv, bden);
+    } else occluded = wave_leaves<ANY, NREC>(tris, O, D, tnear, L, nl, bt, bp, bu, bv, bden);
   }
   return occluded;
 }
@@ -149,7 +153,7 @@
   return (unsigned)__builtin_amdgcn_readfirstlane((int)r) + gridDim.x * 4u;
 }
 
-template <bool XFORM, bool MULTI = false>
+template <bool XFORM, bool MULTI = false, bool NREC = false>
 __global__ __launch_bounds__(256) void k_long_closest(RayPlanes q, const LongRec *__restrict__ recs, const unsigned *__restrict__ n_recs, Mat4 minv,
                                                        Trav T, float tnear, gvt_hip_hit *__restrict__ hits, unsigned *counter, WaveSet W = WaveSet{},
                                                        const int *__restrict__ stk = nullptr, const int *__restrict__ hop_inst = nullptr) {
@@ -198,8 +202,9 @@
       ns = __popcll(mi); nl = __popcll(ml);
     } else if (lane == 0) { s_ref[0] = 0; s_tn[0] = 0.f; }
     __builtin_amdgcn_wave_barrier();
-    wave_run<false, false, LONG_CAP, LONG_PHYS>(T.nodes4, T.tris, O, D, S, tnear, WaveLists{ s_ref, s_tn, l_ref, l_tn }, ns, nl, bt, bp, bu, bv, bden, counter + (CW_TRAV_OVF - CW_LONG_WORK));
-    { gvt_hip_hit h; h.t = bt; h.prim = bp; h.u = (bp >= 0) ? bu / bden : 0.f; h.v = (bp >= 0) ? bv / bden : 0.f; hits[R.j] = h; }
+    wave_run<false, false, LONG_CAP, LONG_PHYS, NREC>(T.nodes4, T.tris, O, D, S, tnear, WaveLists{ s_ref, s_tn, l_ref, l_tn }, ns, nl, bt, bp, bu, bv, bden, counter + (CW_TRAV_OVF - CW_LONG_WORK));
+    if constexpr (NREC) ((float4 *)hits)[R.j] = make_float4(bp >= 0 ? bt : -1.0f, bu, bv, bden);
+    else { gvt_hip_hit h; h.t = bt; h.prim = bp; h.u = (bp >= 0) ? bu / bden : 0.f; h.v = (bp >= 0) ? bv / bden : 0.f; hits[R.j] = h; }
   }
 }
 
diff --git a/include/gvt_hip.h b/include/gvt_hip.h
--- a/include/gvt_hip.h
+++ b/include/gvt_hip.h
@@ -199,6 +199,7 @@
   uint64_t exchanges;
   uint64_t rays_inline;
   uint64_t early_deposit_launches;
+  uint64_t normal_record_launches;
 } gvt_hip_frame_stats;
 int gvt_hip_tracer_frame(gvt_hip_tracer *, int flags, gvt_hip_frame_stats *stats);
 
```

After: 2523 Mrays/s, median of 6. No clear change (+0.6%).
